# apelykh/deep-audio-mixer

Measured on AMD Instinct MI355X. Metric: stem-spectrogram-frames/sec (train), higher is better.
Workload: dtype f32; 1 GPU; C3: model_resnet (ResNet18, 8 stems) train step incl. STFT front-end, 8-stem 3 s @ 44.1 kHz stereo clips, n_fft 2048 hop 1024 -> 8x1025x130 per clip; batch_per_gpu=8, global_batch=8, parallelism=dp1, hip_graph=True, world_size=1, device_index=0, grad_buckets=1, allreduce_overlap=False

## Files before the change

### deep-audio-mixer_amd/csrc/dam_common.h

```cpp
#pragma once
#include <hip/hip_runtime.h>
#include <stdint.h>
#include "dam_hip.h"

#define DAM_CHECK_LAUNCH()                                   \
    do {                                                     \
        if (hipGetLastError() != hipSuccess) return DAM_ERR_LAUNCH; \
    } while (0)

namespace dam {

constexpr int WAVE = 64;

typedef float f32x4 __attribute__((ext_vector_type(4)));
typedef float f32x2 __attribute__((ext_vector_type(2)));
typedef float f32x4_u __attribute__((ext_vector_type(4), aligned(4)));
typedef double f64x2_u __attribute__((ext_vector_type(2), aligned(8)));

__device__ __forceinline__ float2 cmul(float2 a, float2 b) {
    return make_float2(a.x * b.x - a.y * b.y, a.x * b.y + a.y * b.x);
}
__device__ __forceinline__ float2 cadd(float2 a, float2 b) { return make_float2(a.x + b.x, a.y + b.y); }
__device__ __forceinline__ float2 csub(float2 a, float2 b) { return make_float2(a.x - b.x, a.y - b.y); }

__device__ __forceinline__ void wave_lds_sync() {
    __builtin_amdgcn_fence(__ATOMIC_RELEASE, "workgroup");
    __builtin_amdgcn_wave_barrier();
    __builtin_amdgcn_fence(__ATOMIC_ACQUIRE, "workgroup");
}

__device__ __forceinline__ void wave_lds_order() {
    asm volatile("s_waitcnt lgkmcnt(0)" ::: "memory");
    __builtin_amdgcn_wave_barrier();
}

__device__ __forceinline__ float wave_sum16(float v) {
    v += __shfl_xor(v, 1);
    v += __shfl_xor(v, 2);
    v += __shfl_xor(v, 4);
    v += __shfl_xor(v, 8);
    return v;
}
__device__ __forceinline__ float wave_sum64(float v) {
    v = wave_sum16(v);
    v += __shfl_xor(v, 16);
    v += __shfl_xor(v, 32);
    return v;
}

static inline int64_t cdiv(int64_t a, int64_t b) { return (a + b - 1) / b; }

constexpr int BN_RECORDS_MAX = 2048;
constexpr int BN_BWD_RECORDS_MAX = 1024;

struct BnFinArgs {
    const float* gamma;
    const float* beta;
    float* running_mean;
    float* running_var;
    long long* num_batches;
    float momentum, eps;
    float* save_mean;
    float* save_invstd;
    float* scale;
    float* shift;
};

__device__ __forceinline__ void store_sc1(float* p, float v) {
    __hip_atomic_store(p, v, __ATOMIC_RELAXED, __HIP_MEMORY_SCOPE_AGENT);
}

constexpr int MAX_DEVICES = 32;
static inline int device_slot() {
    int d = 0;
    if (hipGetDevice(&d) != hipSuccess || d < 0) d = 0;
    return d % MAX_DEVICES;
}
template <class T>
struct PerDevice {
    T v[MAX_DEVICES] = {};
    T& operator()() { return v[device_slot()]; }
};
template <auto Kernel>
static inline bool raise_lds_limit(int bytes) {
    static PerDevice<bool> raised_pd;
    bool& raised = raised_pd();
    if (!raised)
        raised = hipFuncSetAttribute(reinterpret_cast<const void*>(Kernel), hipFuncAttributeMaxDynamicSharedMemorySize, bytes) == hipSuccess;
    return raised;
}
static inline int device_cus() {
    static PerDevice<int> cus;
    int& n = cus();
    if (!n) {
        int dev = 0;
        if (hipGetDevice(&dev) != hipSuccess || hipDeviceGetAttribute(&n, hipDeviceAttributeMultiprocessorCount, dev) != hipSuccess || n < 1) n = 256;
    }
    return n;
}

}
```

### deep-audio-mixer_amd/csrc/dam_conv_s2.hip

```cpp
#include "dam_common.h"

namespace dam {
namespace {

typedef float v4f __attribute__((ext_vector_type(4)));

template <int NB, int NCH, bool STATS, int WAVES>
__global__ __launch_bounds__(64 * WAVES) void conv_s2_pair_kernel(const float* __restrict__ X, unsigned x_bytes, const float4* __restrict__ Wp,
                                                           const float4* __restrict__ Wp2, int Hd, int Wd, int H, int W,
                                                           float* __restrict__ Y, float* __restrict__ Ys, float* __restrict__ P1,
                                                           float* __restrict__ P2, int total_px, int total_units) {
    extern __shared__ __attribute__((aligned(16))) unsigned char smem[];
    constexpr int Ci = 16 * NCH, Co = 16 * NB;
    static_assert(NCH == 1 || NCH == 2, "the operand sets alternate per chunk (NCH == 2) or per unit (NCH == 1)");
    const int tid = threadIdx.x, lane = tid & 63, wave = tid >> 6;
    const int j = lane & 15, kq = lane >> 4;
    const __amdgpu_buffer_rsrc_t xr = __builtin_amdgcn_make_buffer_rsrc(const_cast<float*>(X), 0, x_bytes, 0x00020000);
    const int w_lane = lane * 16;
    float4 xs[2][9], wa[2][NB];
    v4f acc1[NB], accs[NB];
    float k1[STATS ? NB : 1][4], s11[STATS ? NB : 1][4], s21[STATS ? NB : 1][4];
    float ks[STATS ? NB : 1][4], s1s[STATS ? NB : 1][4], s2s[STATS ? NB : 1][4];
    int n_px = 0;
#pragma unroll
    for (int nb = 0; nb < NB; ++nb) {
        acc1[nb] = (v4f){0.f, 0.f, 0.f, 0.f};
        accs[nb] = (v4f){0.f, 0.f, 0.f, 0.f};
    }
    if constexpr (STATS) {
#pragma unroll
        for (int nb = 0; nb < NB; ++nb)
#pragma unroll
            for (int q = 0; q < 4; ++q) { k1[nb][q] = s11[nb][q] = s21[nb][q] = 0.f; ks[nb][q] = s1s[nb][q] = s2s[nb][q] = 0.f; }
    }
#define DAM_CS2_OFFS(U_, BASE_, FL_)                                                                                          \
    do {                                                                                                                      \
        const int p_ = (U_) * 16 + j;                                                                                         \
        const int row_ = p_ / Wd, col_ = p_ - row_ * Wd, img_ = row_ / Hd, i_ = row_ - img_ * Hd;                             \
        BASE_ = (((img_ * H + 2 * i_) * W + 2 * col_) * Ci + kq * 4) * 4;                                                     \
        FL_ = ((U_) < unit_end && p_ < total_px)                                                                             \
                  ? (1 | (i_ > 0 ? 2 : 0) | (2 * i_ + 1 < H ? 4 : 0) | (col_ > 0 ? 8 : 0) | (2 * col_ + 1 < W ? 16 : 0))      \
                  : 0;                                                                                                        \
    } while (0)
#define DAM_CS2_LOAD(S_, BASE_, FL_, CH_)                                                                                     \
    _Pragma("unroll") for (int a = 0; a < 3; ++a) {                                                                           \
        _Pragma("unroll") for (int b = 0; b < 3; ++b) {                                                                       \
            const int need = 1 | (a == 0 ? 2 : a == 2 ? 4 : 0) | (b == 0 ? 8 : b == 2 ? 16 : 0);                              \
            const int off = ((FL_) & need) == need ? (BASE_) + ((a - 1) * W + (b - 1)) * (Ci * 4) : 0x7fffffff;               \
            xs[S_][a * 3 + b] = __builtin_bit_cast(float4, __builtin_amdgcn_raw_buffer_load_b128(xr, off, (CH_) * 64, 0));    \
        }                                                                                                                     \
    }
#define DAM_CS2_MFMA4(ACC_, WA_, XV_)                                                                                         \
    do {                                                                                                                      \
        ACC_ = __builtin_amdgcn_mfma_f32_16x16x4f32(WA_.x, XV_.x, ACC_, 0, 0, 0);                                             \
        ACC_ = __builtin_amdgcn_mfma_f32_16x16x4f32(WA_.y, XV_.y, ACC_, 0, 0, 0);                                             \
        ACC_ = __builtin_amdgcn_mfma_f32_16x16x4f32(WA_.z, XV_.z, ACC_, 0, 0, 0);                                             \
        ACC_ = __builtin_amdgcn_mfma_f32_16x16x4f32(WA_.w, XV_.w, ACC_, 0, 0, 0);                                             \
    } while (0)
#define DAM_CS2_WREAD(BUF_, T_, CH_)                                                                                          \
    _Pragma("unroll") for (int nb = 0; nb < NB; ++nb)                                                                         \
        wa[BUF_][nb] = *reinterpret_cast<const float4*>(smem + w_lane + (((T_) * NCH + (CH_)) * NB + nb) * 1024);
#define DAM_CS2_COMPUTE(S_, CH_)                                                                                              \
    do {                                                                                                                      \
        DAM_CS2_WREAD(0, 0, CH_)                                                                                              \
        _Pragma("unroll") for (int t = 0; t < 10; ++t) {                                                                      \
            if (t < 9) { DAM_CS2_WREAD((t + 1) & 1, t + 1, CH_) }                                                             \
            __builtin_amdgcn_sched_barrier(0);                                                                                \
                                 \
            _Pragma("unroll") for (int q = 0; q < 4; ++q) {                                                                   \
                _Pragma("unroll") for (int nb = 0; nb < NB; ++nb) {                                                           \
                    const float wq = q == 0 ? wa[t & 1][nb].x : q == 1 ? wa[t & 1][nb].y : q == 2 ? wa[t & 1][nb].z : wa[t & 1][nb].w; \
                    const float4 xv = xs[S_][t < 9 ? t : 4];                                                                  \
                    const float xq = q == 0 ? xv.x : q == 1 ? xv.y : q == 2 ? xv.z : xv.w;                                    \
                    if (t < 9) acc1[nb] = __builtin_amdgcn_mfma_f32_16x16x4f32(wq, xq, acc1[nb], 0, 0, 0);                    \
                    else accs[nb] = __builtin_amdgcn_mfma_f32_16x16x4f32(wq, xq, accs[nb], 0, 0, 0);                          \
                }                                                                                                             \
            }                                                                                                                 \
            __builtin_amdgcn_sched_barrier(0);                                                                                \
        }                                                                                                                     \
    } while (0)
#define DAM_CS2_EPILOGUE(U_)                                                                                                  \
    do {                                                                                                                      \
        const int p_ = (U_) * 16 + j;                                                                                         \
        if (p_ < total_px) {                                                                                                  \
            float* o1 = Y + (size_t)p_ * Co + kq * 4;                                                                         \
            float* o2 = Ys + (size_t)p_ * Co + kq * 4;                                                                        \
            _Pragma("unroll") for (int nb = 0; nb < NB; ++nb) {                                                               \
                *reinterpret_cast<v4f*>(o1 + nb * 16) = acc1[nb];                                                             \
                *reinterpret_cast<v4f*>(o2 + nb * 16) = accs[nb];                                                             \
            }                                                                                                                 \
            if constexpr (STATS) {                                                                                            \
                _Pragma("unroll") for (int nb = 0; nb < NB; ++nb) {                                                           \
                    _Pragma("unroll") for (int q = 0; q < 4; ++q) {                                                           \
                        if (n_px == 0) { k1[nb][q] = acc1[nb][q]; ks[nb][q] = accs[nb][q]; }                                  \
                        const float d1 = acc1[nb][q] - k1[nb][q], d2 = accs[nb][q] - ks[nb][q];                               \
                        s11[nb][q] += d1; s21[nb][q] = fmaf(d1, d1, s21[nb][q]);                                              \
                        s1s[nb][q] += d2; s2s[nb][q] = fmaf(d2, d2, s2s[nb][q]);                                              \
                    }                                                                                                         \
                }                                                                                                             \
                ++n_px;                                                                                                       \
            }                                                                                                                 \
        }                                                                                                                     \
        _Pragma("unroll") for (int nb = 0; nb < NB; ++nb) {                                                                   \
            acc1[nb] = (v4f){0.f, 0.f, 0.f, 0.f};                                                                             \
            accs[nb] = (v4f){0.f, 0.f, 0.f, 0.f};                                                                             \
        }                                                                                                                     \
    } while (0)

    const int n_xcd = (gridDim.x & 7) == 0 ? 8 : 1;
    const int wg_per_xcd = gridDim.x / n_xcd, per_xcd = (total_units + n_xcd - 1) / n_xcd;
    const int u_lo = (blockIdx.x % n_xcd) * per_xcd;
    const int unit_end = u_lo + per_xcd < total_units ? u_lo + per_xcd : total_units;
    const int ustride = wg_per_xcd * WAVES;
    int unit = u_lo + wave * wg_per_xcd + blockIdx.x / n_xcd;
    int base0, fl0, base1, fl1;
    DAM_CS2_OFFS(unit, base0, fl0);
    DAM_CS2_LOAD(0, base0, fl0, 0)
    {
        constexpr int N4 = 9 * NCH * NB * 64, N4P = NCH * NB * 64;
        for (int e = tid; e < N4; e += 64 * WAVES) reinterpret_cast<float4*>(smem)[e] = Wp[e];
        for (int e = tid; e < N4P; e += 64 * WAVES) reinterpret_cast<float4*>(smem)[N4 + e] = Wp2[e];
    }
    __syncthreads();
    while (unit < unit_end) {
        if constexpr (NCH == 2) {
            DAM_CS2_LOAD(1, base0, fl0, 1)
            DAM_CS2_OFFS(unit + ustride, base1, fl1);
            __builtin_amdgcn_sched_barrier(0);
            DAM_CS2_COMPUTE(0, 0);
            __builtin_amdgcn_sched_barrier(0);
            DAM_CS2_LOAD(0, base1, fl1, 0)
            __builtin_amdgcn_sched_barrier(0);
            DAM_CS2_COMPUTE(1, 1);
            __builtin_amdgcn_sched_barrier(0);
            DAM_CS2_EPILOGUE(unit);
            unit += ustride;
            base0 = base1; fl0 = fl1;
        } else {
            const int u1 = unit + ustride, u2 = u1 + ustride;
            DAM_CS2_OFFS(u1, base1, fl1);
            DAM_CS2_LOAD(1, base1, fl1, 0)
            __builtin_amdgcn_sched_barrier(0);
            DAM_CS2_COMPUTE(0, 0);
            __builtin_amdgcn_sched_barrier(0);
            DAM_CS2_EPILOGUE(unit);
            DAM_CS2_OFFS(u2, base0, fl0);
            DAM_CS2_LOAD(0, base0, fl0, 0)
            __builtin_amdgcn_sched_barrier(0);
            if (u1 < unit_end) {
                DAM_CS2_COMPUTE(1, 0);
                __builtin_amdgcn_sched_barrier(0);
                DAM_CS2_EPILOGUE(u1);
            }
            unit = u2;
        }
    }
#undef DAM_CS2_OFFS
#undef DAM_CS2_LOAD
#undef DAM_CS2_MFMA4
#undef DAM_CS2_COMPUTE
#undef DAM_CS2_WREAD
#undef DAM_CS2_EPILOGUE
    if constexpr (STATS) {
        float cnt = (float)n_px;
        const float inv = n_px ? 1.0f / cnt : 0.f;
        float mean1[NB][4], m21[NB][4], means[NB][4], m2s[NB][4];
#pragma unroll
        for (int nb = 0; nb < NB; ++nb)
#pragma unroll
            for (int q = 0; q < 4; ++q) {
                const float a = s11[nb][q] * inv, b = s1s[nb][q] * inv;
                mean1[nb][q] = n_px ? k1[nb][q] + a : 0.f;
                m21[nb][q] = n_px ? fmaxf(s21[nb][q] - s11[nb][q] * a, 0.f) : 0.f;
                means[nb][q] = n_px ? ks[nb][q] + b : 0.f;
                m2s[nb][q] = n_px ? fmaxf(s2s[nb][q] - s1s[nb][q] * b, 0.f) : 0.f;
            }
#pragma unroll
        for (int off = 1; off < 16; off <<= 1) {
            const float cb = __shfl_xor(cnt, off), nn = cnt + cb;
            const float r = nn > 0.f ? cb / nn : 0.f, f = cnt * r;
#pragma unroll
            for (int nb = 0; nb < NB; ++nb)
#pragma unroll
                for (int q = 0; q < 4; ++q) {
                    float mb = __shfl_xor(mean1[nb][q], off), qb = __shfl_xor(m21[nb][q], off), d = mb - mean1[nb][q];
                    mean1[nb][q] = fmaf(d, r, mean1[nb][q]);
                    m21[nb][q] += qb + d * d * f;
                    mb = __shfl_xor(means[nb][q], off); qb = __shfl_xor(m2s[nb][q], off); d = mb - means[nb][q];
                    means[nb][q] = fmaf(d, r, means[nb][q]);
                    m2s[nb][q] += qb + d * d * f;
                }
            cnt = nn;
        }
        __syncthreads();
        float* rec = reinterpret_cast<float*>(smem);
        if (j == 0) {
#pragma unroll
            for (int nb = 0; nb < NB; ++nb)
#pragma unroll
                for (int q = 0; q < 4; ++q) {
                    float* o1 = rec + ((wave * 2 + 0) * Co + nb * 16 + kq * 4 + q) * 3;
                    float* o2 = rec + ((wave * 2 + 1) * Co + nb * 16 + kq * 4 + q) * 3;
                    o1[0] = cnt; o1[1] = mean1[nb][q]; o1[2] = m21[nb][q];
                    o2[0] = cnt; o2[1] = means[nb][q]; o2[2] = m2s[nb][q];
                }
        }
        __syncthreads();
        if (tid < 2 * Co) {
            const int which = tid / Co, c = tid - which * Co;
            float n = 0.f, mean = 0.f, m2 = 0.f;
#pragma unroll
            for (int w = 0; w < WAVES; ++w) {
                const float* r = rec + ((w * 2 + which) * Co + c) * 3;
                const float nb_ = r[0], nn = n + nb_, rr = nn > 0.f ? nb_ / nn : 0.f, d = r[1] - mean;
                mean = fmaf(d, rr, mean);
                m2 += r[2] + d * d * (n * rr);
                n = nn;
            }
            float* o = (which ? P2 : P1) + ((size_t)blockIdx.x * Co + c) * 3;
            o[0] = n; o[1] = mean; o[2] = m2;
        }
    }
}

template <int NB, int NCH, int WAVES>
int launch_conv_s2_pair(const float* x, const float* wp, const float* wp2, int B, int H, int W, float* y, float* ys, float* p1,
                        float* p2, int* parts_host, hipStream_t st) {
    const int Hd = (H + 1) / 2, Wd = (W + 1) / 2;
    const int64_t px = (int64_t)B * Hd * Wd, xb = (int64_t)B * H * W * NCH * 64;
    if (px >= (1ll << 26) || xb >= (1ll << 31)) return DAM_ERR_UNSUPPORTED;
    const int64_t units = cdiv(px, 16);
    const size_t lds = (size_t)10 * NCH * NB * 1024;
    const int cus = device_cus();
    const bool stats = p1 != nullptr;
    static PerDevice<int> occ[2];
    int& oc = occ[stats ? 1 : 0]();
    if (!oc) {
        int n = 0;
        const hipError_t e = stats ? hipOccupancyMaxActiveBlocksPerMultiprocessor(&n, conv_s2_pair_kernel<NB, NCH, true, WAVES>, 64 * WAVES, lds)
                                   : hipOccupancyMaxActiveBlocksPerMultiprocessor(&n, conv_s2_pair_kernel<NB, NCH, false, WAVES>, 64 * WAVES, lds);
        oc = (e == hipSuccess && n >= 1) ? n : 1;
    }
    int max_per_cu = oc;
    if (max_per_cu > 3) max_per_cu = 3;
    if (WAVES == 8) max_per_cu = 1;
    if (max_per_cu < 1) max_per_cu = 1;
    while (max_per_cu > 1 && (int64_t)cus * max_per_cu > BN_RECORDS_MAX) --max_per_cu;
    if ((int64_t)cus > BN_RECORDS_MAX) return DAM_ERR_UNSUPPORTED;
    int per_cu = 1;
    int64_t best = 0;
    for (int n = 1; n <= max_per_cu; ++n) {
        const int64_t cost = cdiv(units, (int64_t)WAVES * cus * n) * n * 100;
        if (n == 1 || cost * 100 <= best * 115) { best = n == 1 ? cost : (cost < best ? cost : best); per_cu = n; }
    }
    int64_t wgs = (int64_t)cus * per_cu;
    if (wgs > cdiv(units, WAVES)) wgs = cdiv(units, WAVES);
    if (parts_host) *parts_host = stats ? (int)wgs : 0;
    if (lds > 64 * 1024 && !(stats ? raise_lds_limit<&conv_s2_pair_kernel<NB, NCH, true, WAVES>>(160 * 1024)
                                   : raise_lds_limit<&conv_s2_pair_kernel<NB, NCH, false, WAVES>>(160 * 1024))) return DAM_ERR_LAUNCH;
    if (stats)
        hipLaunchKernelGGL((conv_s2_pair_kernel<NB, NCH, true, WAVES>), dim3((unsigned)wgs), dim3(64 * WAVES), lds, st, x, (unsigned)xb,
                           reinterpret_cast<const float4*>(wp), reinterpret_cast<const float4*>(wp2), Hd, Wd, H, W, y, ys, p1, p2, (int)px,
                           (int)units);
    else
        hipLaunchKernelGGL((conv_s2_pair_kernel<NB, NCH, false, WAVES>), dim3((unsigned)wgs), dim3(64 * WAVES), lds, st, x, (unsigned)xb,
                           reinterpret_cast<const float4*>(wp), reinterpret_cast<const float4*>(wp2), Hd, Wd, H, W, y, ys, p1, p2, (int)px,
                           (int)units);
    DAM_CHECK_LAUNCH();
    return DAM_OK;
}


template <bool STATS>
__global__ __launch_bounds__(256) void conv_s2_pair_stream_kernel(const float* __restrict__ X, unsigned x_bytes, const float4* __restrict__ Wp,
                                                                  const float4* __restrict__ Wp2, int Hd, int Wd, int H, int W, int NCH,
                                                                  int NB, float* __restrict__ Y, float* __restrict__ Ys,
                                                                  float* __restrict__ P1, float* __restrict__ P2, int total_px) {
    __shared__ float rec[4][2][16][3];
    const int tid = threadIdx.x, lane = tid & 63, wave = tid >> 6;
    const int j = lane & 15, kq = lane >> 4;
    constexpr int MB = 1;
    const int xcd = blockIdx.x & 7, seq = blockIdx.x >> 3;
    const int nb = seq % NB, pgroup = (seq / NB) * 8 + xcd;
    if (pgroup * (64 * MB) >= total_px) return;
    const int Ci = 16 * NCH, Co = 16 * NB;
    const __amdgpu_buffer_rsrc_t xr = __builtin_amdgcn_make_buffer_rsrc(const_cast<float*>(X), 0, x_bytes, 0x00020000);
    int pix[MB], off[MB][9];
#pragma unroll
    for (int mb = 0; mb < MB; ++mb) {
        const int p = ((pgroup * 4 + wave) * MB + mb) * 16 + j;
        pix[mb] = p;
        const int row = p / Wd, col = p - row * Wd, img = row / Hd, i = row - img * Hd;
        const int base = (((img * H + 2 * i) * W + 2 * col) * Ci + kq * 4) * 4;
        const int fl = p < total_px ? (1 | (i > 0 ? 2 : 0) | (2 * i + 1 < H ? 4 : 0) | (col > 0 ? 8 : 0) | (2 * col + 1 < W ? 16 : 0)) : 0;
#pragma unroll
        for (int a = 0; a < 3; ++a)
#pragma unroll
            for (int b = 0; b < 3; ++b) {
                const int need = 1 | (a == 0 ? 2 : a == 2 ? 4 : 0) | (b == 0 ? 8 : b == 2 ? 16 : 0);
                off[mb][a * 3 + b] = (fl & need) == need ? base + ((a - 1) * W + (b - 1)) * (Ci * 4) : 0x7fffffff;
            }
    }
    __shared__ float4 wbuf[2][10 * 64];
    float4 xs[2][MB][9], wa[2], wr0, wr1, wr2;
    const int we0 = tid, we1 = tid + 256, we2 = tid < 128 ? tid + 512 : 0;
#define DAM_CS2S_WSRC(E_, CH_)                                                                                               \
    ((E_) < 576 ? Wp + ((size_t)(((E_) >> 6) * NCH + (CH_)) * NB + nb) * 64 + ((E_) & 63)                                     \
                : Wp2 + ((size_t)(CH_) * NB + nb) * 64 + ((E_) & 63))
#define DAM_CS2S_WFETCH(CH_)                                                                                                  \
    do {                                                                                                                      \
        wr0 = *DAM_CS2S_WSRC(we0, CH_); wr1 = *DAM_CS2S_WSRC(we1, CH_); wr2 = *DAM_CS2S_WSRC(we2, CH_);                       \
    } while (0)
#define DAM_CS2S_WSTORE(BUF_)                                                                                                 \
    do {                                                                                                                      \
        wbuf[BUF_][we0] = wr0; wbuf[BUF_][we1] = wr1;                                                                         \
        if (tid < 128) wbuf[BUF_][we2] = wr2;                                                                                 \
    } while (0)
#define DAM_CS2S_XLOAD(S_, CH_)                                                                                               \
    _Pragma("unroll") for (int mb = 0; mb < MB; ++mb)                                                                         \
        _Pragma("unroll") for (int t = 0; t < 9; ++t)                                                                         \
            xs[S_][mb][t] = __builtin_bit_cast(float4, __builtin_amdgcn_raw_buffer_load_b128(xr, off[mb][t], (CH_) * 64, 0));
#define DAM_CS2S_CHUNK(S_, BUF_)                                                                                              \
    do {                                                                                                                      \
        wa[0] = wbuf[BUF_][lane];                                                                                             \
        _Pragma("unroll") for (int t = 0; t < 10; ++t) {                                                                      \
            if (t < 9) wa[(t + 1) & 1] = wbuf[BUF_][(t + 1) * 64 + lane];                                                     \
            __builtin_amdgcn_sched_barrier(0);                                                                                \
            const float4 w_ = wa[t & 1];                                                                                      \
            _Pragma("unroll") for (int mb = 0; mb < MB; ++mb) {                                                               \
                const float4 x_ = xs[S_][mb][t < 9 ? t : 4];                                                                  \
                if (t < 9) {                                                                                                  \
                    acc1[mb] = __builtin_amdgcn_mfma_f32_16x16x4f32(w_.x, x_.x, acc1[mb], 0, 0, 0);                           \
                    acc1[mb] = __builtin_amdgcn_mfma_f32_16x16x4f32(w_.y, x_.y, acc1[mb], 0, 0, 0);                           \
                    acc1[mb] = __builtin_amdgcn_mfma_f32_16x16x4f32(w_.z, x_.z, acc1[mb], 0, 0, 0);                           \
                    acc1[mb] = __builtin_amdgcn_mfma_f32_16x16x4f32(w_.w, x_.w, acc1[mb], 0, 0, 0);                           \
                } else {                                                                                                      \
                    accs[mb] = __builtin_amdgcn_mfma_f32_16x16x4f32(w_.x, x_.x, accs[mb], 0, 0, 0);                           \
                    accs[mb] = __builtin_amdgcn_mfma_f32_16x16x4f32(w_.y, x_.y, accs[mb], 0, 0, 0);                           \
                    accs[mb] = __builtin_amdgcn_mfma_f32_16x16x4f32(w_.z, x_.z, accs[mb], 0, 0, 0);                           \
                    accs[mb] = __builtin_amdgcn_mfma_f32_16x16x4f32(w_.w, x_.w, accs[mb], 0, 0, 0);                           \
                }                                                                                                             \
            }                                                                                                                 \
            __builtin_amdgcn_sched_barrier(0);                                                                                \
        }                                                                                                                     \
    } while (0)
    v4f acc1[MB], accs[MB];
#pragma unroll
    for (int mb = 0; mb < MB; ++mb) { acc1[mb] = (v4f){0.f, 0.f, 0.f, 0.f}; accs[mb] = (v4f){0.f, 0.f, 0.f, 0.f}; }
    DAM_CS2S_XLOAD(0, 0)
    DAM_CS2S_WFETCH(0);
    DAM_CS2S_WSTORE(0);
    __syncthreads();
    for (int c = 0; c < NCH; c += 2) {
        DAM_CS2S_XLOAD(1, c + 1)
        DAM_CS2S_WFETCH(c + 1);
        __builtin_amdgcn_sched_barrier(0);
        DAM_CS2S_CHUNK(0, 0);
        __builtin_amdgcn_sched_barrier(0);
        DAM_CS2S_WSTORE(1);
        __syncthreads();
        if (c + 2 < NCH) {
            DAM_CS2S_XLOAD(0, c + 2)
            DAM_CS2S_WFETCH(c + 2);
        }
        __builtin_amdgcn_sched_barrier(0);
        DAM_CS2S_CHUNK(1, 1);
        __builtin_amdgcn_sched_barrier(0);
        if (c + 2 < NCH) { DAM_CS2S_WSTORE(0); }
        __syncthreads();
    }
#undef DAM_CS2S_WSRC
#undef DAM_CS2S_WFETCH
#undef DAM_CS2S_WSTORE
#undef DAM_CS2S_XLOAD
#undef DAM_CS2S_CHUNK
#pragma unroll
    for (int mb = 0; mb < MB; ++mb)
        if (pix[mb] < total_px) {
            *reinterpret_cast<v4f*>(Y + (size_t)pix[mb] * Co + nb * 16 + kq * 4) = acc1[mb];
            *reinterpret_cast<v4f*>(Ys + (size_t)pix[mb] * Co + nb * 16 + kq * 4) = accs[mb];
        }
    if constexpr (STATS) {
        float cnt = 0.f;
#pragma unroll
        for (int mb = 0; mb < MB; ++mb) cnt += pix[mb] < total_px ? 1.f : 0.f;
#pragma unroll
        for (int o = 1; o < 16; o <<= 1) cnt += __shfl_xor(cnt, o);
        const float inv = cnt > 0.f ? 1.f / cnt : 0.f;
        float mean[2][4], m2[2][4];
#pragma unroll
        for (int q = 0; q < 4; ++q) {
            float s1 = 0.f, s2 = 0.f;
#pragma unroll
            for (int mb = 0; mb < MB; ++mb)
                if (pix[mb] < total_px) { s1 += acc1[mb][q]; s2 += accs[mb][q]; }
#pragma unroll
            for (int o = 1; o < 16; o <<= 1) { s1 += __shfl_xor(s1, o); s2 += __shfl_xor(s2, o); }
            mean[0][q] = s1 * inv; mean[1][q] = s2 * inv;
            float d1 = 0.f, d2 = 0.f;
#pragma unroll
            for (int mb = 0; mb < MB; ++mb)
                if (pix[mb] < total_px) {
                    const float e1 = acc1[mb][q] - mean[0][q], e2 = accs[mb][q] - mean[1][q];
                    d1 = fmaf(e1, e1, d1); d2 = fmaf(e2, e2, d2);
                }
#pragma unroll
            for (int o = 1; o < 16; o <<= 1) { d1 += __shfl_xor(d1, o); d2 += __shfl_xor(d2, o); }
            m2[0][q] = d1; m2[1][q] = d2;
        }
        if (j == 0) {
#pragma unroll
            for (int q = 0; q < 4; ++q) {
                rec[wave][0][kq * 4 + q][0] = cnt; rec[wave][0][kq * 4 + q][1] = mean[0][q]; rec[wave][0][kq * 4 + q][2] = m2[0][q];
                rec[wave][1][kq * 4 + q][0] = cnt; rec[wave][1][kq * 4 + q][1] = mean[1][q]; rec[wave][1][kq * 4 + q][2] = m2[1][q];
            }
        }
        __syncthreads();
        if (tid < 32) {
            const int which = tid >> 4, c = tid & 15;
            float n = 0.f, mu = 0.f, q2 = 0.f;
#pragma unroll
            for (int w = 0; w < 4; ++w) {
                const float nw = rec[w][which][c][0], nn = n + nw, rr = nn > 0.f ? nw / nn : 0.f, d = rec[w][which][c][1] - mu;
                mu = fmaf(d, rr, mu);
                q2 += rec[w][which][c][2] + d * d * (n * rr);
                n = nn;
            }
            float* o = (which ? P2 : P1) + ((size_t)pgroup * Co + nb * 16 + c) * 3;
            o[0] = n; o[1] = mu; o[2] = q2;
        }
    }
}

int launch_conv_s2_pair_stream(const float* x, const float* wp, const float* wp2, int B, int H, int W, int Ci, int Co, float* y, float* ys,
                               float* p1, float* p2, int* parts_host, hipStream_t st) {
    const int Hd = (H + 1) / 2, Wd = (W + 1) / 2, NCH = Ci / 16, NB = Co / 16;
    const int64_t px = (int64_t)B * Hd * Wd, xb = (int64_t)B * H * W * Ci * 4;
    const int64_t groups = cdiv(px, 64);
    if (px >= (1ll << 26) || xb >= (1ll << 31) || groups * NB >= (1ll << 31) || (int64_t)9 * Ci * Co * 4 >= (1ll << 31)) return DAM_ERR_UNSUPPORTED;
    const bool stats = p1 != nullptr;
    if (stats && groups > BN_RECORDS_MAX) return DAM_ERR_UNSUPPORTED;
    if (parts_host) *parts_host = stats ? (int)groups : 0;
    const dim3 grid((unsigned)(cdiv(groups, 8) * 8 * NB)), block(256);
#define DAM_CS2S_GO(ST_)                                                                                                        \
    hipLaunchKernelGGL((conv_s2_pair_stream_kernel<ST_>), grid, block, 0, st, x, (unsigned)xb, reinterpret_cast<const float4*>(wp), \
                       reinterpret_cast<const float4*>(wp2), Hd, Wd, H, W, NCH, NB, y, ys, p1, p2, (int)px)
    if (stats) DAM_CS2S_GO(true); else DAM_CS2S_GO(false);
#undef DAM_CS2S_GO
    DAM_CHECK_LAUNCH();
    return DAM_OK;
}

}
}

extern "C" int dam_conv_s2_pair_fwd_f32(const float* x, const float* w_packed, const float* wsc_packed, int B, int H, int W, int Ci,
                                        int Co, float* y, float* ysc, float* partial, float* partial_sc, int* parts_host,
                                        void* stream) {
    using namespace dam;
    if (!x || !w_packed || !wsc_packed || !y || !ysc || B <= 0 || H <= 0 || W <= 0) return DAM_ERR_BAD_ARG;
    if ((partial != nullptr) != (partial_sc != nullptr)) return DAM_ERR_BAD_ARG;
    if (partial && !parts_host) return DAM_ERR_BAD_ARG;
    hipStream_t st = (hipStream_t)stream;
    if (Ci == 16 && Co == 32) return launch_conv_s2_pair<2, 1, 4>(x, w_packed, wsc_packed, B, H, W, y, ysc, partial, partial_sc, parts_host, st);
    if (Ci == 32 && Co == 64) return launch_conv_s2_pair<4, 2, 8>(x, w_packed, wsc_packed, B, H, W, y, ysc, partial, partial_sc, parts_host, st);
    if (Ci % 32 == 0 && Co % 16 == 0)
        return launch_conv_s2_pair_stream(x, w_packed, wsc_packed, B, H, W, Ci, Co, y, ysc, partial, partial_sc, parts_host, st);
    return DAM_ERR_UNSUPPORTED;
}
```

### deep-audio-mixer_amd/csrc/dam_dgrad_s2.hip

```cpp
#include "dam_common.h"

namespace dam {
namespace {

typedef float v4f __attribute__((ext_vector_type(4)));

struct S2Sums {
    const float* u; const unsigned char* bits; const float* mean; const float* invstd; float* rec;
};
template <int NB, int NCH, int MB, bool PAIR, int WAVES, bool SUMS>
__global__ __launch_bounds__(64 * WAVES) void dgrad_s2_kernel(const float* __restrict__ DC, const float4* __restrict__ Wp,
                                                       const float* __restrict__ DS, const float4* __restrict__ Wp2, int B, int Hd,
                                                       int Wd, float* __restrict__ DX, int H, int W, int total_px, int total_units,
                                                       const S2Sums sums) {
    extern __shared__ __attribute__((aligned(16))) unsigned char smem[];
    constexpr int Co = 16 * NCH, Ci = 16 * NB;
    const int tid = threadIdx.x, lane = tid & 63, wave = tid >> 6;
    const int j = lane & 15, kq = lane >> 4;
    const __amdgpu_buffer_rsrc_t cr = __builtin_amdgcn_make_buffer_rsrc(const_cast<float*>(DC), 0, (unsigned)((size_t)B * Hd * Wd * Co * 4), 0x00020000);
    const __amdgpu_buffer_rsrc_t sr = __builtin_amdgcn_make_buffer_rsrc(const_cast<float*>(PAIR ? DS : DC), 0, (unsigned)((size_t)B * Hd * Wd * Co * 4), 0x00020000);
    const int w_lane = lane * 16;
    float su1[SUMS ? NB : 1][4], su2[SUMS ? NB : 1][4];
    float4 umu[SUMS ? NB : 1], uis[SUMS ? NB : 1];
    if constexpr (SUMS) {
#pragma unroll
        for (int nb = 0; nb < NB; ++nb) {
            umu[nb] = *reinterpret_cast<const float4*>(sums.mean + nb * 16 + kq * 4);
            uis[nb] = *reinterpret_cast<const float4*>(sums.invstd + nb * 16 + kq * 4);
#pragma unroll
            for (int q = 0; q < 4; ++q) su1[nb][q] = su2[nb][q] = 0.f;
        }
    }
    static_assert(NCH % 2 == 0, "chunk c of every unit uses operand set c & 1");
    float4 xo[2][PAIR ? 5 : 4][MB], wa[2][NB];
    int o00[MB], o01[MB], o10[MB], o11[MB], n00[MB], n01[MB], n10[MB], n11[MB];
#define DAM_S2_OFFSETS(U_, A_, B_, C_, D_)                                                                                    \
    do {                                                                                                                      \
        _Pragma("unroll") for (int mb = 0; mb < MB; ++mb) {                                                                   \
            const int p_ = (U_) * (16 * MB) + mb * 16 + j;              \
            const int row_ = p_ / Wd, col_ = p_ - row_ * Wd, i_ = row_ % Hd;                                                  \
            const int base = (p_ * Co + kq * 4) * 4;                                                                          \
            const bool c0 = (U_) < unit_end && p_ < total_px,    c1 = c0 && col_ + 1 < Wd, row1_ = i_ + 1 < Hd;               \
            A_[mb] = c0 ? base : 0x7fffffff;                                                                                  \
            B_[mb] = c1 ? base + Co * 4 : 0x7fffffff;                                                                         \
            C_[mb] = (c0 && row1_) ? base + Wd * Co * 4 : 0x7fffffff;                                                         \
            D_[mb] = (c1 && row1_) ? base + (Wd + 1) * Co * 4 : 0x7fffffff;                                                   \
        }                                                                                                                     \
    } while (0)
#define DAM_S2_LOAD(S_, A_, B_, C_, D_, CH_)                                                                                  \
    _Pragma("unroll") for (int mb = 0; mb < MB; ++mb) {                                                                       \
        xo[S_][0][mb] = __builtin_bit_cast(float4, __builtin_amdgcn_raw_buffer_load_b128(cr, A_[mb], (CH_) * 64, 0));         \
        xo[S_][1][mb] = __builtin_bit_cast(float4, __builtin_amdgcn_raw_buffer_load_b128(cr, B_[mb], (CH_) * 64, 0));         \
        xo[S_][2][mb] = __builtin_bit_cast(float4, __builtin_amdgcn_raw_buffer_load_b128(cr, C_[mb], (CH_) * 64, 0));         \
        xo[S_][3][mb] = __builtin_bit_cast(float4, __builtin_amdgcn_raw_buffer_load_b128(cr, D_[mb], (CH_) * 64, 0));         \
        if constexpr (PAIR) xo[S_][4][mb] = __builtin_bit_cast(float4, __builtin_amdgcn_raw_buffer_load_b128(sr, A_[mb], (CH_) * 64, 0)); \
    }
    constexpr int NT = PAIR ? 10 : 9;
    constexpr int TAPS[10][3] = {{4, 0, 0}, {3, 1, 1}, {5, 1, 0}, {1, 2, 2}, {7, 2, 0}, {0, 3, 3}, {2, 3, 2}, {6, 3, 1}, {8, 3, 0}, {9, 0, 4}};
#define DAM_S2_WREAD(BUF_, T_, CH_)                                                                                           \
    _Pragma("unroll") for (int nb = 0; nb < NB; ++nb)                                                                         \
        wa[BUF_][nb] = *reinterpret_cast<const float4*>(smem + w_lane + (((T_) * NCH + (CH_)) * NB + nb) * 1024);
#define DAM_S2_CHUNK(S_, CH_)                                                                                                 \
    do {                                                                                                                      \
        DAM_S2_WREAD(0, TAPS[0][0], CH_)                                                                                      \
        _Pragma("unroll") for (int s = 0; s < NT; ++s) {                                                                      \
            if (s + 1 < NT) { DAM_S2_WREAD((s + 1) & 1, TAPS[s + 1 < NT ? s + 1 : 0][0], CH_) }                               \
            __builtin_amdgcn_sched_barrier(0);                                                                                \
                           \
            _Pragma("unroll") for (int q = 0; q < 4; ++q) {                                                                   \
                _Pragma("unroll") for (int nb = 0; nb < NB; ++nb) {                                                           \
                    _Pragma("unroll") for (int mb = 0; mb < MB; ++mb) {                                                       \
                        v4f& a_ = acc[TAPS[s][1]][mb][nb];                                                                    \
                        const float4 w_ = wa[s & 1][nb], x_ = xo[S_][TAPS[s][2]][mb];                                         \
                        const float wq = q == 0 ? w_.x : q == 1 ? w_.y : q == 2 ? w_.z : w_.w;                                \
                        const float xq = q == 0 ? x_.x : q == 1 ? x_.y : q == 2 ? x_.z : x_.w;                                \
                        a_ = __builtin_amdgcn_mfma_f32_16x16x4f32(wq, xq, a_, 0, 0, 0);                                       \
                    }                                                                                                         \
                }                                                                                                             \
            }                                                                                                                 \
            __builtin_amdgcn_sched_barrier(0);                                                                                \
        }                                                                                                                     \
    } while (0)
    const int n_xcd = (gridDim.x & 7) == 0 ? 8 : 1;
    const int wg_per_xcd = gridDim.x / n_xcd, per_xcd = (total_units + n_xcd - 1) / n_xcd;
    const int u_lo = (blockIdx.x % n_xcd) * per_xcd;
    const int unit_end = u_lo + per_xcd < total_units ? u_lo + per_xcd : total_units;
    const int ustride = wg_per_xcd * WAVES;
    int unit = u_lo + wave * wg_per_xcd + blockIdx.x / n_xcd;
    DAM_S2_OFFSETS(unit, o00, o01, o10, o11);
    DAM_S2_LOAD(0, o00, o01, o10, o11, 0)
    {
        constexpr int N4 = 9 * NCH * NB * 64, N4P = PAIR ? NCH * NB * 64 : 0;
        for (int e = tid; e < N4; e += 64 * WAVES) reinterpret_cast<float4*>(smem)[e] = Wp[e];
        if constexpr (PAIR)
            for (int e = tid; e < N4P; e += 64 * WAVES) reinterpret_cast<float4*>(smem)[N4 + e] = Wp2[e];
    }
    __syncthreads();
    while (unit < unit_end) {
        v4f acc[4][MB][NB];
#pragma unroll
        for (int cl = 0; cl < 4; ++cl)
#pragma unroll
            for (int mb = 0; mb < MB; ++mb)
#pragma unroll
                for (int nb = 0; nb < NB; ++nb) acc[cl][mb][nb] = (v4f){0.f, 0.f, 0.f, 0.f};
        DAM_S2_OFFSETS(unit + ustride, n00, n01, n10, n11);
        float4 uv[SUMS ? MB : 1][4][NB];
        unsigned ub[SUMS ? MB : 1][4][NB];
#pragma unroll
        for (int c = 0; c < NCH; ++c) {
            if (c + 1 < NCH) { DAM_S2_LOAD((c + 1) & 1, o00, o01, o10, o11, c + 1) }
            else { DAM_S2_LOAD(0, n00, n01, n10, n11, 0) }
            if constexpr (SUMS) {
                if (c == NCH - 1) {
#pragma unroll
                    for (int mb = 0; mb < MB; ++mb) {
                        const int p = unit * (16 * MB) + mb * 16 + j;
                        const int row = p / Wd, col = p - row * Wd, img = row / Hd, i = row - img * Hd;
                        const bool live = p < total_px, orow1 = 2 * i + 1 < H, ocol1 = 2 * col + 1 < W;
                        const size_t px00 = ((size_t)img * H + 2 * i) * W + 2 * col;
#pragma unroll
                        for (int cl = 0; cl < 4; ++cl) {
                            const bool ok = live && (cl & 1 ? ocol1 : true) && (cl & 2 ? orow1 : true);
                            const size_t px = px00 + (cl & 1 ? 1 : 0) + (cl & 2 ? (size_t)W : 0);
#pragma unroll
                            for (int nb = 0; nb < NB; ++nb) {
                                uv[mb][cl][nb] = ok ? *reinterpret_cast<const float4*>(sums.u + px * Ci + nb * 16 + kq * 4) : make_float4(0.f, 0.f, 0.f, 0.f);
                                ub[mb][cl][nb] = ok ? sums.bits[px * (Ci / 4) + nb * 4 + kq] : 0u;
                            }
                        }
                    }
                }
            }
            __builtin_amdgcn_sched_barrier(0);
            DAM_S2_CHUNK(c & 1, c);
            __builtin_amdgcn_sched_barrier(0);
        }
#pragma unroll
        for (int mb = 0; mb < MB; ++mb) {
            const int p = unit * (16 * MB) + mb * 16 + j;
            if (p >= total_px) continue;
            const int row = p / Wd, col = p - row * Wd, img = row / Hd, i = row - img * Hd;
            const bool orow1 = 2 * i + 1 < H, ocol1 = 2 * col + 1 < W;
            const size_t px00 = ((size_t)img * H + 2 * i) * W + 2 * col;
            const size_t p00 = px00 * Ci + kq * 4;
            if constexpr (SUMS) {
#pragma unroll
                for (int nb = 0; nb < NB; ++nb) {
                    float* o = DX + p00 + nb * 16;
                    *reinterpret_cast<v4f*>(o) = acc[0][mb][nb];
                    if (ocol1) *reinterpret_cast<v4f*>(o + Ci) = acc[1][mb][nb];
                    if (orow1) {
                        *reinterpret_cast<v4f*>(o + (size_t)W * Ci) = acc[2][mb][nb];
                        if (ocol1) *reinterpret_cast<v4f*>(o + (size_t)W * Ci + Ci) = acc[3][mb][nb];
                    }
                }
#pragma unroll
                for (int cl = 0; cl < 4; ++cl)
#pragma unroll
                    for (int nb = 0; nb < NB; ++nb) {
                        const float uq[4] = {uv[mb][cl][nb].x, uv[mb][cl][nb].y, uv[mb][cl][nb].z, uv[mb][cl][nb].w};
                        const float mq[4] = {umu[nb].x, umu[nb].y, umu[nb].z, umu[nb].w}, iq[4] = {uis[nb].x, uis[nb].y, uis[nb].z, uis[nb].w};
#pragma unroll
                        for (int q = 0; q < 4; ++q) {
                            const float dz = (ub[mb][cl][nb] >> q) & 1u ? acc[cl][mb][nb][q] : 0.f;
                            su1[nb][q] += dz;
                            su2[nb][q] = fmaf(dz, (uq[q] - mq[q]) * iq[q], su2[nb][q]);
                        }
                    }
            } else {
#pragma unroll
                for (int nb = 0; nb < NB; ++nb) {
                    float* o = DX + p00 + nb * 16;
                    *reinterpret_cast<v4f*>(o) = acc[0][mb][nb];
                    if (ocol1) *reinterpret_cast<v4f*>(o + Ci) = acc[1][mb][nb];
                    if (orow1) {
                        *reinterpret_cast<v4f*>(o + (size_t)W * Ci) = acc[2][mb][nb];
                        if (ocol1) *reinterpret_cast<v4f*>(o + (size_t)W * Ci + Ci) = acc[3][mb][nb];
                    }
                }
            }
        }
        unit += ustride;
#pragma unroll
        for (int mb = 0; mb < MB; ++mb) { o00[mb] = n00[mb]; o01[mb] = n01[mb]; o10[mb] = n10[mb]; o11[mb] = n11[mb]; }
    }
    if constexpr (SUMS) {
#pragma unroll
        for (int off = 1; off < 16; off <<= 1)
#pragma unroll
            for (int nb = 0; nb < NB; ++nb)
#pragma unroll
                for (int q = 0; q < 4; ++q) { su1[nb][q] += __shfl_xor(su1[nb][q], off); su2[nb][q] += __shfl_xor(su2[nb][q], off); }
        __syncthreads();
        float* red = reinterpret_cast<float*>(smem);
        if (j == 0) {
#pragma unroll
            for (int nb = 0; nb < NB; ++nb)
#pragma unroll
                for (int q = 0; q < 4; ++q) {
                    red[(wave * Ci + nb * 16 + kq * 4 + q) * 2] = su1[nb][q];
                    red[(wave * Ci + nb * 16 + kq * 4 + q) * 2 + 1] = su2[nb][q];
                }
        }
        __syncthreads();
        if (tid < 2 * Ci) {
            float t = 0.f;
#pragma unroll
            for (int w = 0; w < WAVES; ++w) t += red[w * Ci * 2 + tid];
            sums.rec[(size_t)blockIdx.x * Ci * 2 + tid] = t;
        }
    }
#undef DAM_S2_OFFSETS
#undef DAM_S2_LOAD
#undef DAM_S2_WREAD
#undef DAM_S2_CHUNK
}

template <int NB, int NCH, int MB, int WAVES>
int launch_dgrad_s2(const float* dc, const float* wpt, const float* ds, const float* wpt2, int B, int Hd, int Wd, float* dx, int H,
                    int W, const S2Sums& sums, int* parts_host, hipStream_t st) {
    const int64_t px = (int64_t)B * Hd * Wd;
    if (px >= (1ll << 30)) return DAM_ERR_UNSUPPORTED;
    const int64_t units = cdiv(px, 16 * MB);
    const size_t lds = (size_t)(9 + (ds ? 1 : 0)) * NCH * NB * 1024;
    const int cus = device_cus();
    static PerDevice<int> occ[2][2];
    int& oc = occ[ds ? 1 : 0][sums.u ? 1 : 0]();
    if (!oc) {
        int n = 0;
        hipError_t e;
        if (ds) e = sums.u ? hipOccupancyMaxActiveBlocksPerMultiprocessor(&n, dgrad_s2_kernel<NB, NCH, MB, true, WAVES, true>, 64 * WAVES, lds)
                           : hipOccupancyMaxActiveBlocksPerMultiprocessor(&n, dgrad_s2_kernel<NB, NCH, MB, true, WAVES, false>, 64 * WAVES, lds);
        else e = sums.u ? hipOccupancyMaxActiveBlocksPerMultiprocessor(&n, dgrad_s2_kernel<NB, NCH, MB, false, WAVES, true>, 64 * WAVES, lds)
                        : hipOccupancyMaxActiveBlocksPerMultiprocessor(&n, dgrad_s2_kernel<NB, NCH, MB, false, WAVES, false>, 64 * WAVES, lds);
        oc = (e == hipSuccess && n >= 1) ? n : 1;
    }
    int max_per_cu = oc;
    if (max_per_cu > 3) max_per_cu = 3;
    if (WAVES == 8) max_per_cu = 1;
    int per_cu = 1;
    int64_t best = 0;
    for (int n = 1; n <= max_per_cu; ++n) {
        const int64_t cost = cdiv(units, (int64_t)WAVES * cus * n) * n * 100;
        if (n == 1 || cost * 100 <= best * 115) { best = n == 1 ? cost : (cost < best ? cost : best); per_cu = n; }
    }
    int64_t wgs = (int64_t)cus * per_cu;
    if (wgs > cdiv(units, WAVES)) wgs = cdiv(units, WAVES);
    if (sums.u && wgs > BN_BWD_RECORDS_MAX) return DAM_ERR_UNSUPPORTED;
#define DAM_S2_GO(PAIR_, SUMS_)                                                                                                   \
    do {                                                                                                                          \
        if (lds > 64 * 1024 && !raise_lds_limit<&dgrad_s2_kernel<NB, NCH, MB, PAIR_, WAVES, SUMS_>>(160 * 1024)) return DAM_ERR_LAUNCH; \
        hipLaunchKernelGGL((dgrad_s2_kernel<NB, NCH, MB, PAIR_, WAVES, SUMS_>), dim3((unsigned)wgs), dim3(64 * WAVES), lds, st, dc, \
                           reinterpret_cast<const float4*>(wpt), ds, reinterpret_cast<const float4*>(wpt2), B, Hd, Wd, dx, H, W,      \
                           (int)px, (int)units, sums);                                                                            \
    } while (0)
    if (ds) { if (sums.u) DAM_S2_GO(true, true); else DAM_S2_GO(true, false); }
    else { if (sums.u) DAM_S2_GO(false, true); else DAM_S2_GO(false, false); }
#undef DAM_S2_GO
    if (parts_host) *parts_host = sums.u ? (int)wgs : 0;
    DAM_CHECK_LAUNCH();
    return DAM_OK;
}


template <bool PAIR>
__global__ __launch_bounds__(256) void dgrad_s2_stream_kernel(const float* __restrict__ DC, const float4* __restrict__ Wp,
                                                              const float* __restrict__ DS, const float4* __restrict__ Wp2, int Hd, int Wd,
                                                              float* __restrict__ DX, int H, int W, int total_px, int NCH, int NB,
                                                              int total_units) {
    constexpr int MB = 2;
    const int lane = threadIdx.x & 63, wave = threadIdx.x >> 6;
    const int unit = blockIdx.x * 4 + wave;
    if (unit >= total_units) return;
    const int nb = unit % NB, pg = unit / NB;
    const int j = lane & 15, kq = lane >> 4;
    const int Co = 16 * NCH, Ci = 16 * NB;
    const __amdgpu_buffer_rsrc_t cr = __builtin_amdgcn_make_buffer_rsrc(const_cast<float*>(DC), 0, (unsigned)((size_t)total_px * Co * 4), 0x00020000);
    const __amdgpu_buffer_rsrc_t sr = __builtin_amdgcn_make_buffer_rsrc(const_cast<float*>(PAIR ? DS : DC), 0, (unsigned)((size_t)total_px * Co * 4), 0x00020000);
    const __amdgpu_buffer_rsrc_t wr = __builtin_amdgcn_make_buffer_rsrc(const_cast<float4*>(Wp), 0, (unsigned)((size_t)9 * NCH * NB * 1024), 0x00020000);
    const __amdgpu_buffer_rsrc_t w2r = __builtin_amdgcn_make_buffer_rsrc(const_cast<float4*>(PAIR ? Wp2 : Wp), 0, (unsigned)((size_t)NCH * NB * 1024), 0x00020000);
    int o00[MB], o01[MB], o10[MB], o11[MB];
#pragma unroll
    for (int mb = 0; mb < MB; ++mb) {
        const int p = pg * (16 * MB) + mb * 16 + j;
        const int row = p / Wd, col = p - row * Wd, i = row % Hd;
        const int base = (p * Co + kq * 4) * 4;
        const bool c0 = p < total_px, c1 = c0 && col + 1 < Wd, row1 = i + 1 < Hd;
        o00[mb] = c0 ? base : 0x7fffffff;
        o01[mb] = c1 ? base + Co * 4 : 0x7fffffff;
        o10[mb] = (c0 && row1) ? base + Wd * Co * 4 : 0x7fffffff;
        o11[mb] = (c1 && row1) ? base + (Wd + 1) * Co * 4 : 0x7fffffff;
    }
    float4 x00[2][MB], x01[2][MB], x10[2][MB], x11[2][MB], s00[2][PAIR ? MB : 1], wt[2][PAIR ? 10 : 9];
#define DAM_S2S_LOAD(S_, CH_)                                                                                                 \
    do {                                                                                                                      \
        _Pragma("unroll") for (int mb = 0; mb < MB; ++mb) {                                                                   \
            x00[S_][mb] = __builtin_bit_cast(float4, __builtin_amdgcn_raw_buffer_load_b128(cr, o00[mb], (CH_) * 64, 0));      \
            x01[S_][mb] = __builtin_bit_cast(float4, __builtin_amdgcn_raw_buffer_load_b128(cr, o01[mb], (CH_) * 64, 0));      \
            x10[S_][mb] = __builtin_bit_cast(float4, __builtin_amdgcn_raw_buffer_load_b128(cr, o10[mb], (CH_) * 64, 0));      \
            x11[S_][mb] = __builtin_bit_cast(float4, __builtin_amdgcn_raw_buffer_load_b128(cr, o11[mb], (CH_) * 64, 0));      \
            if constexpr (PAIR) s00[S_][mb] = __builtin_bit_cast(float4, __builtin_amdgcn_raw_buffer_load_b128(sr, o00[mb], (CH_) * 64, 0)); \
        }                                                                                                                     \
        _Pragma("unroll") for (int t = 0; t < 9; ++t)                                                                         \
            wt[S_][t] = __builtin_bit_cast(float4, __builtin_amdgcn_raw_buffer_load_b128(wr, lane * 16, ((t * NCH + (CH_)) * NB + nb) * 1024, 0)); \
        if constexpr (PAIR)                                                                                                   \
            wt[S_][9] = __builtin_bit_cast(float4, __builtin_amdgcn_raw_buffer_load_b128(w2r, lane * 16, ((CH_) * NB + nb) * 1024, 0)); \
    } while (0)
#define DAM_S2S_TAP(T_, CL_, X_, S_)                                                                                          \
    _Pragma("unroll") for (int mb = 0; mb < MB; ++mb) {                                                                       \
        acc[CL_][mb] = __builtin_amdgcn_mfma_f32_16x16x4f32(wt[S_][T_].x, X_[S_][mb].x, acc[CL_][mb], 0, 0, 0);               \
        acc[CL_][mb] = __builtin_amdgcn_mfma_f32_16x16x4f32(wt[S_][T_].y, X_[S_][mb].y, acc[CL_][mb], 0, 0, 0);               \
        acc[CL_][mb] = __builtin_amdgcn_mfma_f32_16x16x4f32(wt[S_][T_].z, X_[S_][mb].z, acc[CL_][mb], 0, 0, 0);               \
        acc[CL_][mb] = __builtin_amdgcn_mfma_f32_16x16x4f32(wt[S_][T_].w, X_[S_][mb].w, acc[CL_][mb], 0, 0, 0);               \
    }
#define DAM_S2S_CHUNK(S_)                                                                                                     \
    do {                                                                                                                      \
        DAM_S2S_TAP(4, 0, x00, S_)                                                                                            \
        if constexpr (PAIR) { DAM_S2S_TAP(9, 0, s00, S_) }                                                                    \
        DAM_S2S_TAP(3, 1, x01, S_) DAM_S2S_TAP(5, 1, x00, S_)                                                                 \
        DAM_S2S_TAP(1, 2, x10, S_) DAM_S2S_TAP(7, 2, x00, S_)                                                                 \
        DAM_S2S_TAP(0, 3, x11, S_) DAM_S2S_TAP(2, 3, x10, S_) DAM_S2S_TAP(6, 3, x01, S_) DAM_S2S_TAP(8, 3, x00, S_)           \
    } while (0)
    v4f acc[4][MB];
#pragma unroll
    for (int cl = 0; cl < 4; ++cl)
#pragma unroll
        for (int mb = 0; mb < MB; ++mb) acc[cl][mb] = (v4f){0.f, 0.f, 0.f, 0.f};
    DAM_S2S_LOAD(0, 0);
    for (int c = 0; c < NCH; c += 2) {
        DAM_S2S_LOAD(1, c + 1);
        __builtin_amdgcn_sched_barrier(0);
        DAM_S2S_CHUNK(0);
        __builtin_amdgcn_sched_barrier(0);
        if (c + 2 < NCH) DAM_S2S_LOAD(0, c + 2);
        __builtin_amdgcn_sched_barrier(0);
        DAM_S2S_CHUNK(1);
        __builtin_amdgcn_sched_barrier(0);
    }
#pragma unroll
    for (int mb = 0; mb < MB; ++mb) {
        const int p = pg * (16 * MB) + mb * 16 + j;
        if (p >= total_px) continue;
        const int row = p / Wd, col = p - row * Wd, img = row / Hd, i = row - img * Hd;
        const bool orow1 = 2 * i + 1 < H, ocol1 = 2 * col + 1 < W;
        float* o = DX + (((size_t)img * H + 2 * i) * W + 2 * col) * Ci + nb * 16 + kq * 4;
        *reinterpret_cast<v4f*>(o) = acc[0][mb];
        if (ocol1) *reinterpret_cast<v4f*>(o + Ci) = acc[1][mb];
        if (orow1) {
            *reinterpret_cast<v4f*>(o + (size_t)W * Ci) = acc[2][mb];
            if (ocol1) *reinterpret_cast<v4f*>(o + (size_t)W * Ci + Ci) = acc[3][mb];
        }
    }
#undef DAM_S2S_LOAD
#undef DAM_S2S_TAP
#undef DAM_S2S_CHUNK
}

template <bool PAIR>
__global__ __launch_bounds__(256) void dgrad_s2_stream_lds_kernel(const float* __restrict__ DC, const float4* __restrict__ Wp,
                                                                  const float* __restrict__ DS, const float4* __restrict__ Wp2, int Hd,
                                                                  int Wd, float* __restrict__ DX, int H, int W, int total_px, int NCH,
                                                                  int NB) {
    constexpr int NT = PAIR ? 10 : 9, NQ = NT * 64;
    __shared__ float4 wbuf[2][NQ];
    const int tid = threadIdx.x, lane = tid & 63, wave = tid >> 6;
    const int xcd = blockIdx.x & 7, seq = blockIdx.x >> 3;
    const int nb = seq % NB, grp = (seq / NB) * 8 + xcd;
    if (grp * 64 >= total_px) return;
    const int pg = grp * 4 + wave;
    const int j = lane & 15, kq = lane >> 4;
    const int Co = 16 * NCH, Ci = 16 * NB;
    const __amdgpu_buffer_rsrc_t cr = __builtin_amdgcn_make_buffer_rsrc(const_cast<float*>(DC), 0, (unsigned)((size_t)total_px * Co * 4), 0x00020000);
    const __amdgpu_buffer_rsrc_t sr = __builtin_amdgcn_make_buffer_rsrc(const_cast<float*>(PAIR ? DS : DC), 0, (unsigned)((size_t)total_px * Co * 4), 0x00020000);
    const int p = pg * 16 + j;
    const int row = p / Wd, col = p - row * Wd, img = row / Hd, i = row - img * Hd;
    int ov[4];
    {
        const int base = (p * Co + kq * 4) * 4;
        const bool c0 = p < total_px, c1 = c0 && col + 1 < Wd, row1 = i + 1 < Hd;
        ov[0] = c0 ? base : 0x7fffffff;
        ov[1] = c1 ? base + Co * 4 : 0x7fffffff;
        ov[2] = (c0 && row1) ? base + Wd * Co * 4 : 0x7fffffff;
        ov[3] = (c1 && row1) ? base + (Wd + 1) * Co * 4 : 0x7fffffff;
    }
    float4 xo[2][PAIR ? 5 : 4], wa[2], wr0, wr1, wr2;
    const int we0 = tid, we1 = tid + 256, we2 = tid + 512 < NQ ? tid + 512 : 0;
#define DAM_S2L_WSRC(E_, CH_)                                                                                                \
    ((E_) < 576 ? Wp + ((size_t)(((E_) >> 6) * NCH + (CH_)) * NB + nb) * 64 + ((E_) & 63)                                     \
                : Wp2 + ((size_t)(CH_) * NB + nb) * 64 + ((E_) & 63))
#define DAM_S2L_WFETCH(CH_)                                                                                                   \
    do {                                                                                                                      \
        wr0 = *DAM_S2L_WSRC(we0, CH_); wr1 = *DAM_S2L_WSRC(we1, CH_); wr2 = *DAM_S2L_WSRC(we2, CH_);                          \
    } while (0)
#define DAM_S2L_WSTORE(BUF_)                                                                                                  \
    do {                                                                                                                      \
        wbuf[BUF_][we0] = wr0; wbuf[BUF_][we1] = wr1;                                                                         \
        if (tid + 512 < NQ) wbuf[BUF_][we2] = wr2;                                                                            \
    } while (0)
#define DAM_S2L_XLOAD(S_, CH_)                                                                                                \
    do {                                                                                                                      \
        _Pragma("unroll") for (int v = 0; v < 4; ++v)                                                                         \
            xo[S_][v] = __builtin_bit_cast(float4, __builtin_amdgcn_raw_buffer_load_b128(cr, ov[v], (CH_) * 64, 0));          \
        if constexpr (PAIR) xo[S_][4] = __builtin_bit_cast(float4, __builtin_amdgcn_raw_buffer_load_b128(sr, ov[0], (CH_) * 64, 0)); \
    } while (0)
    constexpr int TAPS[10][3] = {{4, 0, 0}, {3, 1, 1}, {5, 1, 0}, {1, 2, 2}, {7, 2, 0}, {0, 3, 3}, {2, 3, 2}, {6, 3, 1}, {8, 3, 0}, {9, 0, 4}};
#define DAM_S2L_CHUNK(S_, BUF_)                                                                                               \
    do {                                                                                                                      \
        wa[0] = wbuf[BUF_][TAPS[0][0] * 64 + lane];                                                                           \
        _Pragma("unroll") for (int s = 0; s < NT; ++s) {                                                                      \
            if (s + 1 < NT) wa[(s + 1) & 1] = wbuf[BUF_][TAPS[s + 1 < NT ? s + 1 : 0][0] * 64 + lane];                        \
            __builtin_amdgcn_sched_barrier(0);                                                                                \
            const float4 w_ = wa[s & 1], x_ = xo[S_][TAPS[s][2]];                                                             \
            v4f& a_ = acc[TAPS[s][1]];                                                                                        \
            a_ = __builtin_amdgcn_mfma_f32_16x16x4f32(w_.x, x_.x, a_, 0, 0, 0);                                               \
            a_ = __builtin_amdgcn_mfma_f32_16x16x4f32(w_.y, x_.y, a_, 0, 0, 0);                                               \
            a_ = __builtin_amdgcn_mfma_f32_16x16x4f32(w_.z, x_.z, a_, 0, 0, 0);                                               \
            a_ = __builtin_amdgcn_mfma_f32_16x16x4f32(w_.w, x_.w, a_, 0, 0, 0);                                               \
            __builtin_amdgcn_sched_barrier(0);                                                                                \
        }                                                                                                                     \
    } while (0)
    v4f acc[4];
#pragma unroll
    for (int cl = 0; cl < 4; ++cl) acc[cl] = (v4f){0.f, 0.f, 0.f, 0.f};
    DAM_S2L_XLOAD(0, 0);
    DAM_S2L_WFETCH(0);
    DAM_S2L_WSTORE(0);
    __syncthreads();
    for (int c = 0; c < NCH; c += 2) {
        DAM_S2L_XLOAD(1, c + 1);
        DAM_S2L_WFETCH(c + 1);
        __builtin_amdgcn_sched_barrier(0);
        DAM_S2L_CHUNK(0, 0);
        __builtin_amdgcn_sched_barrier(0);
        DAM_S2L_WSTORE(1);
        __syncthreads();
        if (c + 2 < NCH) {
            DAM_S2L_XLOAD(0, c + 2);
            DAM_S2L_WFETCH(c + 2);
        }
        __builtin_amdgcn_sched_barrier(0);
        DAM_S2L_CHUNK(1, 1);
        __builtin_amdgcn_sched_barrier(0);
        if (c + 2 < NCH) { DAM_S2L_WSTORE(0); }
        __syncthreads();
    }
#undef DAM_S2L_WSRC
#undef DAM_S2L_WFETCH
#undef DAM_S2L_WSTORE
#undef DAM_S2L_XLOAD
#undef DAM_S2L_CHUNK
    if (p < total_px) {
        const bool orow1 = 2 * i + 1 < H, ocol1 = 2 * col + 1 < W;
        float* o = DX + (((size_t)img * H + 2 * i) * W + 2 * col) * Ci + nb * 16 + kq * 4;
        *reinterpret_cast<v4f*>(o) = acc[0];
        if (ocol1) *reinterpret_cast<v4f*>(o + Ci) = acc[1];
        if (orow1) {
            *reinterpret_cast<v4f*>(o + (size_t)W * Ci) = acc[2];
            if (ocol1) *reinterpret_cast<v4f*>(o + (size_t)W * Ci + Ci) = acc[3];
        }
    }
}

int launch_dgrad_s2_stream(const float* dc, const float* wpt, const float* ds, const float* wpt2, int B, int Hd, int Wd, int Co, int Ci,
                           float* dx, int H, int W, hipStream_t st) {
    const int64_t px = (int64_t)B * Hd * Wd;
    const int NCH = Co / 16, NB = Ci / 16;
    const int MB = cdiv(px, 16) * NB >= 8 * 1024 ? 2 : 1;
    const int64_t units = cdiv(px, 16 * MB) * NB;
    if (px >= (1ll << 26) || units >= (1ll << 30)) return DAM_ERR_UNSUPPORTED;
    if (MB == 1) {
        const dim3 grid_l((unsigned)(cdiv(cdiv(px, 64), 8) * 8 * NB)), block_l(256);
        if (ds)
            hipLaunchKernelGGL((dgrad_s2_stream_lds_kernel<true>), grid_l, block_l, 0, st, dc, reinterpret_cast<const float4*>(wpt), ds,
                               reinterpret_cast<const float4*>(wpt2), Hd, Wd, dx, H, W, (int)px, NCH, NB);
        else
            hipLaunchKernelGGL((dgrad_s2_stream_lds_kernel<false>), grid_l, block_l, 0, st, dc, reinterpret_cast<const float4*>(wpt),
                               (const float*)nullptr, (const float4*)nullptr, Hd, Wd, dx, H, W, (int)px, NCH, NB);
        DAM_CHECK_LAUNCH();
        return DAM_OK;
    }
    const dim3 grid((unsigned)cdiv(units, 4)), block(256);
    if (ds)
        hipLaunchKernelGGL((dgrad_s2_stream_kernel<true>), grid, block, 0, st, dc, reinterpret_cast<const float4*>(wpt), ds,
                           reinterpret_cast<const float4*>(wpt2), Hd, Wd, dx, H, W, (int)px, NCH, NB, (int)units);
    else
        hipLaunchKernelGGL((dgrad_s2_stream_kernel<false>), grid, block, 0, st, dc, reinterpret_cast<const float4*>(wpt),
                           (const float*)nullptr, (const float4*)nullptr, Hd, Wd, dx, H, W, (int)px, NCH, NB, (int)units);
    DAM_CHECK_LAUNCH();
    return DAM_OK;
}

}
}

extern "C" int dam_dgrad_s2_3x3_f32(const float* dy, const float* w_packed_t, const float* dy_pair, const float* w_pair_packed_t,
                                    int B, int Hd, int Wd, int Co, int Ci, float* dx, int H, int W, const dam_bn_bwd_sums* bn_bwd,
                                    float* bn_partial, int* bn_parts_host, void* stream) {
    using namespace dam;
    if (!dy || !w_packed_t || !dx || B <= 0 || Hd <= 0 || Wd <= 0 || H <= 0 || W <= 0) return DAM_ERR_BAD_ARG;
    if ((dy_pair != nullptr) != (w_pair_packed_t != nullptr)) return DAM_ERR_BAD_ARG;
    if (Hd != (H + 1) / 2 || Wd != (W + 1) / 2) return DAM_ERR_BAD_ARG;
    if ((int64_t)B * Hd * Wd * Co * 4 >= (1ll << 31)) return DAM_ERR_UNSUPPORTED;
    hipStream_t st = (hipStream_t)stream;
    if (bn_parts_host) *bn_parts_host = 0;
    S2Sums sums{nullptr, nullptr, nullptr, nullptr, nullptr};
    if (bn_bwd && bn_bwd->x && bn_bwd->mask_bits && bn_bwd->mean && bn_bwd->invstd && bn_partial && bn_parts_host)
        sums = S2Sums{bn_bwd->x, bn_bwd->mask_bits, bn_bwd->mean, bn_bwd->invstd, bn_partial};
    if (Co == 32 && Ci == 16) return launch_dgrad_s2<1, 2, 2, 4>(dy, w_packed_t, dy_pair, w_pair_packed_t, B, Hd, Wd, dx, H, W, sums, bn_parts_host, st);
    if (Co == 64 && Ci == 32) return launch_dgrad_s2<2, 4, 1, 8>(dy, w_packed_t, dy_pair, w_pair_packed_t, B, Hd, Wd, dx, H, W, sums, bn_parts_host, st);
    if (Co % 32 == 0 && Ci % 16 == 0 && (int64_t)9 * Co * Ci * 4 < (1ll << 31))
        return launch_dgrad_s2_stream(dy, w_packed_t, dy_pair, w_pair_packed_t, B, Hd, Wd, Co, Ci, dx, H, W, st);
    return DAM_ERR_UNSUPPORTED;
}
```

Before: 2.044 million stem-spectrogram-frames/s.

## Software-pipeline stride-2 conv kernels with deferred stores and magic-number division

Reworks the stride-2 conv forward and dgrad kernels. Output stores and BN-statistics updates for the previous unit are interleaved with the MFMA stream of the current unit using double-buffered accumulators and buffer stores. Accumulator zeroing is folded into the first MFMA, and integer divisions by Wd/Hd are replaced with precomputed multiply-high reciprocals. Pivot selection for statistics now uses DPP row broadcasts. This adds register pressure and scheduling complexity, and the dgrad launcher's size limits are tightened.

```diff
diff --git a/deep-audio-mixer_amd/csrc/dam_common.h b/deep-audio-mixer_amd/csrc/dam_common.h
--- a/deep-audio-mixer_amd/csrc/dam_common.h
+++ b/deep-audio-mixer_amd/csrc/dam_common.h
@@ -50,6 +50,17 @@
 
 static inline int64_t cdiv(int64_t a, int64_t b) { return (a + b - 1) / b; }
 
+struct MulHiDiv {
+    unsigned m, s;
+};
+static inline MulHiDiv mulhi_div(unsigned d) {
+    const unsigned D = 2u * d;
+    unsigned s = 0;
+    while ((2ull << s) < D) ++s;
+    return MulHiDiv{(unsigned)((1ull << (32 + s)) / D) + 1u, s};
+}
+__device__ __forceinline__ int mulhi_div(int n, MulHiDiv f) { return (int)(__umulhi(2u * (unsigned)n + 1u, f.m) >> f.s); }
+
 constexpr int BN_RECORDS_MAX = 2048;
 constexpr int BN_BWD_RECORDS_MAX = 1024;
 
diff --git a/deep-audio-mixer_amd/csrc/dam_conv_s2.hip b/deep-audio-mixer_amd/csrc/dam_conv_s2.hip
--- a/deep-audio-mixer_amd/csrc/dam_conv_s2.hip
+++ b/deep-audio-mixer_amd/csrc/dam_conv_s2.hip
@@ -4,29 +4,45 @@
 namespace {
 
 typedef float v4f __attribute__((ext_vector_type(4)));
+typedef int v4i __attribute__((ext_vector_type(4)));
+
+__device__ __forceinline__ float row_first(float v) {
+    return __builtin_bit_cast(float, __builtin_amdgcn_update_dpp(0, __builtin_bit_cast(int, v), 0x150, 0xF, 0xF, false));
+}
+__device__ __forceinline__ void row_sum(float& v) {
+    v += __builtin_bit_cast(float, __builtin_amdgcn_update_dpp(0, __builtin_bit_cast(int, v), 0x128, 0xF, 0xF, false));
+    v += __builtin_bit_cast(float, __builtin_amdgcn_update_dpp(0, __builtin_bit_cast(int, v), 0x124, 0xF, 0xF, false));
+    v += __builtin_bit_cast(float, __builtin_amdgcn_update_dpp(0, __builtin_bit_cast(int, v), 0x122, 0xF, 0xF, false));
+    v += __builtin_bit_cast(float, __builtin_amdgcn_update_dpp(0, __builtin_bit_cast(int, v), 0x121, 0xF, 0xF, false));
+}
 
 template <int NB, int NCH, bool STATS, int WAVES>
 __global__ __launch_bounds__(64 * WAVES) void conv_s2_pair_kernel(const float* __restrict__ X, unsigned x_bytes, const float4* __restrict__ Wp,
                                                            const float4* __restrict__ Wp2, int Hd, int Wd, int H, int W,
                                                            float* __restrict__ Y, float* __restrict__ Ys, float* __restrict__ P1,
-                                                           float* __restrict__ P2, int total_px, int total_units) {
+                                                           float* __restrict__ P2, int total_px, int total_units,
+                                                           const MulHiDiv div_wd, const MulHiDiv div_hd) {
     extern __shared__ __attribute__((aligned(16))) unsigned char smem[];
     constexpr int Ci = 16 * NCH, Co = 16 * NB;
     static_assert(NCH == 1 || NCH == 2, "the operand sets alternate per chunk (NCH == 2) or per unit (NCH == 1)");
-    const int tid = threadIdx.x, lane = tid & 63, wave = tid >> 6;
+    const int tid = threadIdx.x, lane = tid & 63, wave = __builtin_amdgcn_readfirstlane(tid >> 6);
     const int j = lane & 15, kq = lane >> 4;
     const __amdgpu_buffer_rsrc_t xr = __builtin_amdgcn_make_buffer_rsrc(const_cast<float*>(X), 0, x_bytes, 0x00020000);
     const int w_lane = lane * 16;
     float4 xs[2][9], wa[2][NB];
-    v4f acc1[NB], accs[NB];
+    constexpr int NSET = NCH == 1 ? 2 : 1;
+    v4f acc1[NSET][NB], accs[NSET][NB];
     float k1[STATS ? NB : 1][4], s11[STATS ? NB : 1][4], s21[STATS ? NB : 1][4];
     float ks[STATS ? NB : 1][4], s1s[STATS ? NB : 1][4], s2s[STATS ? NB : 1][4];
     int n_px = 0;
-#pragma unroll
-    for (int nb = 0; nb < NB; ++nb) {
-        acc1[nb] = (v4f){0.f, 0.f, 0.f, 0.f};
-        accs[nb] = (v4f){0.f, 0.f, 0.f, 0.f};
-    }
+    bool have_pivot = false;
+#pragma unroll
+    for (int nb = 0; nb < NB; ++nb)
+#pragma unroll
+        for (int a = 0; a < NSET; ++a) {
+            acc1[a][nb] = (v4f){0.f, 0.f, 0.f, 0.f};
+            accs[a][nb] = (v4f){0.f, 0.f, 0.f, 0.f};
+        }
     if constexpr (STATS) {
 #pragma unroll
         for (int nb = 0; nb < NB; ++nb)
@@ -36,7 +52,7 @@
 #define DAM_CS2_OFFS(U_, BASE_, FL_)                                                                                          \
     do {                                                                                                                      \
         const int p_ = (U_) * 16 + j;                                                                                         \
-        const int row_ = p_ / Wd, col_ = p_ - row_ * Wd, img_ = row_ / Hd, i_ = row_ - img_ * Hd;                             \
+        const int row_ = mulhi_div(p_, div_wd), col_ = p_ - row_ * Wd, img_ = mulhi_div(row_, div_hd), i_ = row_ - img_ * Hd; \
         BASE_ = (((img_ * H + 2 * i_) * W + 2 * col_) * Ci + kq * 4) * 4;                                                     \
         FL_ = ((U_) < unit_end && p_ < total_px)                                                                             \
                   ? (1 | (i_ > 0 ? 2 : 0) | (2 * i_ + 1 < H ? 4 : 0) | (col_ > 0 ? 8 : 0) | (2 * col_ + 1 < W ? 16 : 0))      \
@@ -72,8 +88,8 @@
                     const float wq = q == 0 ? wa[t & 1][nb].x : q == 1 ? wa[t & 1][nb].y : q == 2 ? wa[t & 1][nb].z : wa[t & 1][nb].w; \
                     const float4 xv = xs[S_][t < 9 ? t : 4];                                                                  \
                     const float xq = q == 0 ? xv.x : q == 1 ? xv.y : q == 2 ? xv.z : xv.w;                                    \
-                    if (t < 9) acc1[nb] = __builtin_amdgcn_mfma_f32_16x16x4f32(wq, xq, acc1[nb], 0, 0, 0);                    \
-                    else accs[nb] = __builtin_amdgcn_mfma_f32_16x16x4f32(wq, xq, accs[nb], 0, 0, 0);                          \
+                    if (t < 9) acc1[0][nb] = __builtin_amdgcn_mfma_f32_16x16x4f32(wq, xq, acc1[0][nb], 0, 0, 0);              \
+                    else accs[0][nb] = __builtin_amdgcn_mfma_f32_16x16x4f32(wq, xq, accs[0][nb], 0, 0, 0);                    \
                 }                                                                                                             \
             }                                                                                                                 \
             __builtin_amdgcn_sched_barrier(0);                                                                                \
@@ -82,18 +98,28 @@
 #define DAM_CS2_EPILOGUE(U_)                                                                                                  \
     do {                                                                                                                      \
         const int p_ = (U_) * 16 + j;                                                                                         \
+        if constexpr (STATS) {                                                                                                \
+            if (!have_pivot) {                      \
+                _Pragma("unroll") for (int nb = 0; nb < NB; ++nb) {                                                           \
+                    _Pragma("unroll") for (int q = 0; q < 4; ++q) {                                                           \
+                        k1[nb][q] = row_first(acc1[0][nb][q]);                                                                \
+                        ks[nb][q] = row_first(accs[0][nb][q]);                                                                \
+                    }                                                                                                         \
+                }                                                                                                             \
+                have_pivot = true;                                                                                            \
+            }                                                                                                                 \
+        }                                                                                                                     \
         if (p_ < total_px) {                                                                                                  \
             float* o1 = Y + (size_t)p_ * Co + kq * 4;                                                                         \
             float* o2 = Ys + (size_t)p_ * Co + kq * 4;                                                                        \
             _Pragma("unroll") for (int nb = 0; nb < NB; ++nb) {                                                               \
-                *reinterpret_cast<v4f*>(o1 + nb * 16) = acc1[nb];                                                             \
-                *reinterpret_cast<v4f*>(o2 + nb * 16) = accs[nb];                                                             \
+                *reinterpret_cast<v4f*>(o1 + nb * 16) = acc1[0][nb];                                                          \
+                *reinterpret_cast<v4f*>(o2 + nb * 16) = accs[0][nb];                                                          \
             }                                                                                                                 \
             if constexpr (STATS) {                                                                                            \
                 _Pragma("unroll") for (int nb = 0; nb < NB; ++nb) {                                                           \
                     _Pragma("unroll") for (int q = 0; q < 4; ++q) {                                                           \
-                        if (n_px == 0) { k1[nb][q] = acc1[nb][q]; ks[nb][q] = accs[nb][q]; }                                  \
-                        const float d1 = acc1[nb][q] - k1[nb][q], d2 = accs[nb][q] - ks[nb][q];                               \
+                        const float d1 = acc1[0][nb][q] - k1[nb][q], d2 = accs[0][nb][q] - ks[nb][q];                         \
                         s11[nb][q] += d1; s21[nb][q] = fmaf(d1, d1, s21[nb][q]);                                              \
                         s1s[nb][q] += d2; s2s[nb][q] = fmaf(d2, d2, s2s[nb][q]);                                              \
                     }                                                                                                         \
@@ -102,8 +128,8 @@
             }                                                                                                                 \
         }                                                                                                                     \
         _Pragma("unroll") for (int nb = 0; nb < NB; ++nb) {                                                                   \
-            acc1[nb] = (v4f){0.f, 0.f, 0.f, 0.f};                                                                             \
-            accs[nb] = (v4f){0.f, 0.f, 0.f, 0.f};                                                                             \
+            acc1[0][nb] = (v4f){0.f, 0.f, 0.f, 0.f};                                                                          \
+            accs[0][nb] = (v4f){0.f, 0.f, 0.f, 0.f};                                                                          \
         }                                                                                                                     \
     } while (0)
 
@@ -122,6 +148,104 @@
         for (int e = tid; e < N4P; e += 64 * WAVES) reinterpret_cast<float4*>(smem)[N4 + e] = Wp2[e];
     }
     __syncthreads();
+
+    const __amdgpu_buffer_rsrc_t yr = __builtin_amdgcn_make_buffer_rsrc(Y, 0, (unsigned)total_px * (Co * 4), 0x00020000);
+    const __amdgpu_buffer_rsrc_t ysr = __builtin_amdgcn_make_buffer_rsrc(Ys, 0, (unsigned)total_px * (Co * 4), 0x00020000);
+    int loff[9], bn = 0, fn = 0, e_off = 0x7fffffff;
+    bool e_live = false;
+#define DAM_CS2_TAPOFFS(BASE_, FL_)                                                                                           \
+    _Pragma("unroll") for (int a = 0; a < 3; ++a) {                                                                           \
+        _Pragma("unroll") for (int b = 0; b < 3; ++b) {                                                                       \
+            const int need = 1 | (a == 0 ? 2 : a == 2 ? 4 : 0) | (b == 0 ? 8 : b == 2 ? 16 : 0);                              \
+            loff[a * 3 + b] = ((FL_) & need) == need ? (BASE_) + ((a - 1) * W + (b - 1)) * (Ci * 4) : 0x7fffffff;             \
+        }                                                                                                                     \
+    }
+#define DAM_CS2_LOADX(S_)                                                                                                     \
+    _Pragma("unroll") for (int t = 0; t < 9; ++t)                                                                             \
+        xs[S_][t] = __builtin_bit_cast(float4, __builtin_amdgcn_raw_buffer_load_b128(xr, loff[t], 0, 0));
+#define DAM_CS2_STORES(PS_)                                                                                                   \
+    _Pragma("unroll") for (int nb = 0; nb < NB; ++nb) {                                                                       \
+        __builtin_amdgcn_raw_buffer_store_b128(__builtin_bit_cast(v4i, acc1[PS_][nb]), yr, e_off + nb * 64, 0, 0);                           \
+        __builtin_amdgcn_raw_buffer_store_b128(__builtin_bit_cast(v4i, accs[PS_][nb]), ysr, e_off + nb * 64, 0, 0);                          \
+    }
+#define DAM_CS2_STAT(PS_, V_)                                                                                                 \
+    do {                                                                                                                      \
+        const int nb_ = (V_) >> 2, q_ = (V_) & 3;                                                                             \
+        float d1 = acc1[PS_][nb_][q_] - k1[nb_][q_], d2 = accs[PS_][nb_][q_] - ks[nb_][q_];                                   \
+        d1 = e_live ? d1 : 0.f; d2 = e_live ? d2 : 0.f;                                                                       \
+        s11[nb_][q_] += d1; s21[nb_][q_] = fmaf(d1, d1, s21[nb_][q_]);                                                        \
+        s1s[nb_][q_] += d2; s2s[nb_][q_] = fmaf(d2, d2, s2s[nb_][q_]);                                                        \
+    } while (0)
+#define DAM_CS2_STREAM(S_, PS_, UNN_)                                                                                         \
+    do {                                                                                                                      \
+        DAM_CS2_WREAD(0, 0, 0)                                                                                                \
+        _Pragma("unroll") for (int t = 0; t < 10; ++t) {                                                                      \
+            if (t < 9) { DAM_CS2_WREAD((t + 1) & 1, t + 1, 0) }                                                               \
+            __builtin_amdgcn_sched_barrier(0);                                                                                \
+            _Pragma("unroll") for (int q = 0; q < 4; ++q) {                                                                   \
+                _Pragma("unroll") for (int nb = 0; nb < NB; ++nb) {                                                           \
+                    const float wq = q == 0 ? wa[t & 1][nb].x : q == 1 ? wa[t & 1][nb].y : q == 2 ? wa[t & 1][nb].z : wa[t & 1][nb].w; \
+                    const float4 xv = xs[S_][t < 9 ? t : 4];                                                                  \
+                    const float xq = q == 0 ? xv.x : q == 1 ? xv.y : q == 2 ? xv.z : xv.w;                                    \
+                    const v4f zero = {0.f, 0.f, 0.f, 0.f};                                                                    \
+                    if (t < 9) acc1[S_][nb] = __builtin_amdgcn_mfma_f32_16x16x4f32(wq, xq, t == 0 && q == 0 ? zero : acc1[S_][nb], 0, 0, 0); \
+                    else accs[S_][nb] = __builtin_amdgcn_mfma_f32_16x16x4f32(wq, xq, q == 0 ? zero : accs[S_][nb], 0, 0, 0);  \
+                }                                                                                                             \
+            }                                                                                                                 \
+            if (t == 0) {                                                                                                     \
+                DAM_CS2_STORES(PS_)                                                                                           \
+                if constexpr (STATS) n_px += e_live ? 1 : 0;                                                                  \
+            }                                                                                                                 \
+            if constexpr (STATS) {                                                                                            \
+                if (t < 8) {                                                                                                  \
+                    _Pragma("unroll") for (int v = t * (NB / 2); v < (t + 1) * (NB / 2); ++v) DAM_CS2_STAT(PS_, v);           \
+                }                                                                                                             \
+            }                                                                                                                 \
+                      \
+            if (t != 4) xs[S_][t == 9 ? 4 : t] = __builtin_bit_cast(float4, __builtin_amdgcn_raw_buffer_load_b128(xr, loff[t == 9 ? 4 : t], 0, 0)); \
+            if (t == 8) DAM_CS2_OFFS(UNN_, bn, fn);                                                                           \
+            if (t == 9) { DAM_CS2_TAPOFFS(bn, fn) }                                                                           \
+                            \
+            _Pragma("unroll") for (int m = 0; m < 4 * NB; ++m) {                                                              \
+                __builtin_amdgcn_sched_group_barrier(0x008, 1, 0);                                                            \
+                __builtin_amdgcn_sched_group_barrier(0x062, 4, 0);                                                            \
+            }                                                                                                                 \
+            __builtin_amdgcn_sched_barrier(0);                                                                                \
+        }                                                                                                                     \
+    } while (0)
+#define DAM_CS2_AFTER(S_, U_)                                                                                                 \
+    do {                                                                                                                      \
+        if constexpr (STATS) {                                                                                                \
+            if (!have_pivot) {                                                                                                \
+                _Pragma("unroll") for (int nb = 0; nb < NB; ++nb) {                                                           \
+                    _Pragma("unroll") for (int q = 0; q < 4; ++q) {                                                           \
+                        k1[nb][q] = row_first(acc1[S_][nb][q]);                                                               \
+                        ks[nb][q] = row_first(accs[S_][nb][q]);                                                               \
+                    }                                                                                                         \
+                }                                                                                                             \
+                have_pivot = true;                                                                                            \
+            }                                                                                                                 \
+        }                                                                                                                     \
+        const int p_ = (U_) * 16 + j;                                                                                         \
+        e_live = p_ < total_px;                                                                                               \
+        e_off = e_live ? (p_ * Co + kq * 4) * 4 : 0x7fffffff;                                                                 \
+    } while (0)
+#define DAM_CS2_DRAIN(PS_)                                                                                                    \
+    do {                                                                                                                      \
+        DAM_CS2_STORES(PS_)                                                                                                   \
+        if constexpr (STATS) {                                                                                                \
+            n_px += e_live ? 1 : 0;                                                                                           \
+            _Pragma("unroll") for (int v = 0; v < 4 * NB; ++v) DAM_CS2_STAT(PS_, v);                                          \
+        }                                                                                                                     \
+    } while (0)
+    if constexpr (NCH == 1) {
+        static_assert(NB % 2 == 0, "DAM_CS2_STREAM spreads the 4 * NB statistics channels over taps 0-7");
+        DAM_CS2_OFFS(unit + ustride, bn, fn);
+        DAM_CS2_TAPOFFS(bn, fn)
+        DAM_CS2_LOADX(1)
+        DAM_CS2_OFFS(unit + 2 * ustride, bn, fn);
+        DAM_CS2_TAPOFFS(bn, fn)
+    }
     while (unit < unit_end) {
         if constexpr (NCH == 2) {
             DAM_CS2_LOAD(1, base0, fl0, 1)
@@ -137,22 +261,14 @@
             unit += ustride;
             base0 = base1; fl0 = fl1;
         } else {
-            const int u1 = unit + ustride, u2 = u1 + ustride;
-            DAM_CS2_OFFS(u1, base1, fl1);
-            DAM_CS2_LOAD(1, base1, fl1, 0)
-            __builtin_amdgcn_sched_barrier(0);
-            DAM_CS2_COMPUTE(0, 0);
-            __builtin_amdgcn_sched_barrier(0);
-            DAM_CS2_EPILOGUE(unit);
-            DAM_CS2_OFFS(u2, base0, fl0);
-            DAM_CS2_LOAD(0, base0, fl0, 0)
-            __builtin_amdgcn_sched_barrier(0);
-            if (u1 < unit_end) {
-                DAM_CS2_COMPUTE(1, 0);
-                __builtin_amdgcn_sched_barrier(0);
-                DAM_CS2_EPILOGUE(u1);
-            }
-            unit = u2;
+            DAM_CS2_STREAM(0, 1, unit + 3 * ustride);
+            DAM_CS2_AFTER(0, unit);
+            unit += ustride;
+            if (unit >= unit_end) { DAM_CS2_DRAIN(0); break; }
+            DAM_CS2_STREAM(1, 0, unit + 3 * ustride);
+            DAM_CS2_AFTER(1, unit);
+            unit += ustride;
+            if (unit >= unit_end) { DAM_CS2_DRAIN(1); break; }
         }
     }
 #undef DAM_CS2_OFFS
@@ -161,37 +277,30 @@
 #undef DAM_CS2_COMPUTE
 #undef DAM_CS2_WREAD
 #undef DAM_CS2_EPILOGUE
+#undef DAM_CS2_TAPOFFS
+#undef DAM_CS2_LOADX
+#undef DAM_CS2_STORES
+#undef DAM_CS2_STAT
+#undef DAM_CS2_STREAM
+#undef DAM_CS2_AFTER
+#undef DAM_CS2_DRAIN
     if constexpr (STATS) {
         float cnt = (float)n_px;
-        const float inv = n_px ? 1.0f / cnt : 0.f;
+        row_sum(cnt);
+        const float inv = cnt > 0.f ? 1.0f / cnt : 0.f;
         float mean1[NB][4], m21[NB][4], means[NB][4], m2s[NB][4];
 #pragma unroll
         for (int nb = 0; nb < NB; ++nb)
 #pragma unroll
             for (int q = 0; q < 4; ++q) {
+                row_sum(s11[nb][q]); row_sum(s21[nb][q]);
+                row_sum(s1s[nb][q]); row_sum(s2s[nb][q]);
                 const float a = s11[nb][q] * inv, b = s1s[nb][q] * inv;
-                mean1[nb][q] = n_px ? k1[nb][q] + a : 0.f;
-                m21[nb][q] = n_px ? fmaxf(s21[nb][q] - s11[nb][q] * a, 0.f) : 0.f;
-                means[nb][q] = n_px ? ks[nb][q] + b : 0.f;
-                m2s[nb][q] = n_px ? fmaxf(s2s[nb][q] - s1s[nb][q] * b, 0.f) : 0.f;
+                mean1[nb][q] = k1[nb][q] + a;
+                m21[nb][q] = fmaxf(s21[nb][q] - s11[nb][q] * a, 0.f);
+                means[nb][q] = ks[nb][q] + b;
+                m2s[nb][q] = fmaxf(s2s[nb][q] - s1s[nb][q] * b, 0.f);
             }
-#pragma unroll
-        for (int off = 1; off < 16; off <<= 1) {
-            const float cb = __shfl_xor(cnt, off), nn = cnt + cb;
-            const float r = nn > 0.f ? cb / nn : 0.f, f = cnt * r;
-#pragma unroll
-            for (int nb = 0; nb < NB; ++nb)
-#pragma unroll
-                for (int q = 0; q < 4; ++q) {
-                    float mb = __shfl_xor(mean1[nb][q], off), qb = __shfl_xor(m21[nb][q], off), d = mb - mean1[nb][q];
-                    mean1[nb][q] = fmaf(d, r, mean1[nb][q]);
-                    m21[nb][q] += qb + d * d * f;
-                    mb = __shfl_xor(means[nb][q], off); qb = __shfl_xor(m2s[nb][q], off); d = mb - means[nb][q];
-                    means[nb][q] = fmaf(d, r, means[nb][q]);
-                    m2s[nb][q] += qb + d * d * f;
-                }
-            cnt = nn;
-        }
         __syncthreads();
         float* rec = reinterpret_cast<float*>(smem);
         if (j == 0) {
@@ -228,7 +337,7 @@
                         float* p2, int* parts_host, hipStream_t st) {
     const int Hd = (H + 1) / 2, Wd = (W + 1) / 2;
     const int64_t px = (int64_t)B * Hd * Wd, xb = (int64_t)B * H * W * NCH * 64;
-    if (px >= (1ll << 26) || xb >= (1ll << 31)) return DAM_ERR_UNSUPPORTED;
+    if (px >= (1ll << 26) || xb >= (1ll << 31) || px * NB * 64 >= (1ll << 31)) return DAM_ERR_UNSUPPORTED;
     const int64_t units = cdiv(px, 16);
     const size_t lds = (size_t)10 * NCH * NB * 1024;
     const int cus = device_cus();
@@ -261,11 +370,11 @@
     if (stats)
         hipLaunchKernelGGL((conv_s2_pair_kernel<NB, NCH, true, WAVES>), dim3((unsigned)wgs), dim3(64 * WAVES), lds, st, x, (unsigned)xb,
                            reinterpret_cast<const float4*>(wp), reinterpret_cast<const float4*>(wp2), Hd, Wd, H, W, y, ys, p1, p2, (int)px,
-                           (int)units);
+                           (int)units, mulhi_div((unsigned)Wd), mulhi_div((unsigned)Hd));
     else
         hipLaunchKernelGGL((conv_s2_pair_kernel<NB, NCH, false, WAVES>), dim3((unsigned)wgs), dim3(64 * WAVES), lds, st, x, (unsigned)xb,
                            reinterpret_cast<const float4*>(wp), reinterpret_cast<const float4*>(wp2), Hd, Wd, H, W, y, ys, p1, p2, (int)px,
-                           (int)units);
+                           (int)units, mulhi_div((unsigned)Wd), mulhi_div((unsigned)Hd));
     DAM_CHECK_LAUNCH();
     return DAM_OK;
 }
diff --git a/deep-audio-mixer_amd/csrc/dam_dgrad_s2.hip b/deep-audio-mixer_amd/csrc/dam_dgrad_s2.hip
--- a/deep-audio-mixer_amd/csrc/dam_dgrad_s2.hip
+++ b/deep-audio-mixer_amd/csrc/dam_dgrad_s2.hip
@@ -4,6 +4,7 @@
 namespace {
 
 typedef float v4f __attribute__((ext_vector_type(4)));
+typedef int v4i __attribute__((ext_vector_type(4)));
 
 struct S2Sums {
     const float* u; const unsigned char* bits; const float* mean; const float* invstd; float* rec;
@@ -12,10 +13,10 @@
 __global__ __launch_bounds__(64 * WAVES) void dgrad_s2_kernel(const float* __restrict__ DC, const float4* __restrict__ Wp,
                                                        const float* __restrict__ DS, const float4* __restrict__ Wp2, int B, int Hd,
                                                        int Wd, float* __restrict__ DX, int H, int W, int total_px, int total_units,
-                                                       const S2Sums sums) {
+                                                       const MulHiDiv div_wd, const MulHiDiv div_hd, const S2Sums sums) {
     extern __shared__ __attribute__((aligned(16))) unsigned char smem[];
     constexpr int Co = 16 * NCH, Ci = 16 * NB;
-    const int tid = threadIdx.x, lane = tid & 63, wave = tid >> 6;
+    const int tid = threadIdx.x, lane = tid & 63, wave = __builtin_amdgcn_readfirstlane(tid >> 6);
     const int j = lane & 15, kq = lane >> 4;
     const __amdgpu_buffer_rsrc_t cr = __builtin_amdgcn_make_buffer_rsrc(const_cast<float*>(DC), 0, (unsigned)((size_t)B * Hd * Wd * Co * 4), 0x00020000);
     const __amdgpu_buffer_rsrc_t sr = __builtin_amdgcn_make_buffer_rsrc(const_cast<float*>(PAIR ? DS : DC), 0, (unsigned)((size_t)B * Hd * Wd * Co * 4), 0x00020000);
@@ -34,12 +35,15 @@
     static_assert(NCH % 2 == 0, "chunk c of every unit uses operand set c & 1");
     float4 xo[2][PAIR ? 5 : 4][MB], wa[2][NB];
     int o00[MB], o01[MB], o10[MB], o11[MB], n00[MB], n01[MB], n10[MB], n11[MB];
-#define DAM_S2_OFFSETS(U_, A_, B_, C_, D_)                                                                                    \
+    int opx[MB], ofl[MB], npx[MB], nfl[MB];
+#define DAM_S2_OFFSETS(U_, A_, B_, C_, D_, PX_, FL_)                                                                          \
     do {                                                                                                                      \
         _Pragma("unroll") for (int mb = 0; mb < MB; ++mb) {                                                                   \
             const int p_ = (U_) * (16 * MB) + mb * 16 + j;              \
-            const int row_ = p_ / Wd, col_ = p_ - row_ * Wd, i_ = row_ % Hd;                                                  \
+            const int row_ = mulhi_div(p_, div_wd), col_ = p_ - row_ * Wd, img_ = mulhi_div(row_, div_hd), i_ = row_ - img_ * Hd; \
             const int base = (p_ * Co + kq * 4) * 4;                                                                          \
+            PX_[mb] = (img_ * H + 2 * i_) * W + 2 * col_;                                                                     \
+            FL_[mb] = (p_ < total_px ? 1 : 0) | (2 * col_ + 1 < W ? 2 : 0) | (2 * i_ + 1 < H ? 4 : 0);                        \
             const bool c0 = (U_) < unit_end && p_ < total_px,    c1 = c0 && col_ + 1 < Wd, row1_ = i_ + 1 < Hd;               \
             A_[mb] = c0 ? base : 0x7fffffff;                                                                                  \
             B_[mb] = c1 ? base + Co * 4 : 0x7fffffff;                                                                         \
@@ -56,27 +60,57 @@
         if constexpr (PAIR) xo[S_][4][mb] = __builtin_bit_cast(float4, __builtin_amdgcn_raw_buffer_load_b128(sr, A_[mb], (CH_) * 64, 0)); \
     }
     constexpr int NT = PAIR ? 10 : 9;
-    constexpr int TAPS[10][3] = {{4, 0, 0}, {3, 1, 1}, {5, 1, 0}, {1, 2, 2}, {7, 2, 0}, {0, 3, 3}, {2, 3, 2}, {6, 3, 1}, {8, 3, 0}, {9, 0, 4}};
+    constexpr int TAPS[10][3] = {{4, 0, 0}, {9, 0, 4}, {3, 1, 1}, {5, 1, 0}, {1, 2, 2}, {7, 2, 0}, {0, 3, 3}, {2, 3, 2}, {6, 3, 1}, {8, 3, 0}};
+    constexpr int T0 = PAIR ? 0 : 1;
+#define DAM_S2_TAP(S_, K_) (TAPS[(S_) == 0 ? 0 : (S_) + T0][K_])
+    static_assert(MB * NB == 2, "DAM_S2_FILL gives each of a class's MB * NB accumulators one of the two taps behind the class");
+    const __amdgpu_buffer_rsrc_t dxr = __builtin_amdgcn_make_buffer_rsrc(DX, 0, (unsigned)((size_t)B * H * W * Ci * 4), 0x00020000);
+#define DAM_S2_ITEM(CL_, MB_, NB_)                                                                                            \
+    do {                                                                                                                      \
+        const int need_ = 1 | ((CL_) & 1 ? 2 : 0) | ((CL_) & 2 ? 4 : 0);                                                      \
+        const int wo_ = (ofl[MB_] & need_) == need_                                                                           \
+                            ? (opx[MB_] + ((CL_) & 1 ? 1 : 0) + ((CL_) & 2 ? W : 0)) * (Ci * 4) + kq * 16 + (NB_) * 64        \
+                            : 0x7fffffff;                                                                                     \
+        __builtin_amdgcn_raw_buffer_store_b128(__builtin_bit_cast(v4i, acc[CL_][MB_][NB_]), dxr, wo_, 0, 0);                  \
+    } while (0)
+#define DAM_S2_FILL(s, CH_)                                                                                                   \
+    if ((CH_) == 0 && s == 0) DAM_S2_OFFSETS(unit + ustride, n00, n01, n10, n11, npx, nfl);                                   \
+    if ((CH_) == NCH - 1) {                                                                                                   \
+        _Pragma("unroll") for (int cl = 0; cl < 3; ++cl) {                                                                    \
+            const int it = s - ((PAIR ? 1 : 0) + 2 * cl) - 1;                                                                 \
+            if (it == 0) DAM_S2_ITEM(cl, 0, 0);                                                                               \
+            if (it == 1) DAM_S2_ITEM(cl, MB - 1, NB - 1);                                                                     \
+        }                                                                                                                     \
+    }
 #define DAM_S2_WREAD(BUF_, T_, CH_)                                                                                           \
     _Pragma("unroll") for (int nb = 0; nb < NB; ++nb)                                                                         \
         wa[BUF_][nb] = *reinterpret_cast<const float4*>(smem + w_lane + (((T_) * NCH + (CH_)) * NB + nb) * 1024);
 #define DAM_S2_CHUNK(S_, CH_)                                                                                                 \
     do {                                                                                                                      \
-        DAM_S2_WREAD(0, TAPS[0][0], CH_)                                                                                      \
+        DAM_S2_WREAD(0, DAM_S2_TAP(0, 0), CH_)                                                                                \
         _Pragma("unroll") for (int s = 0; s < NT; ++s) {                                                                      \
-            if (s + 1 < NT) { DAM_S2_WREAD((s + 1) & 1, TAPS[s + 1 < NT ? s + 1 : 0][0], CH_) }                               \
+            if (s + 1 < NT) { DAM_S2_WREAD((s + 1) & 1, DAM_S2_TAP(s + 1 < NT ? s + 1 : 0, 0), CH_) }                         \
             __builtin_amdgcn_sched_barrier(0);                                                                                \
-                           \
+             \
+                                                                 \
             _Pragma("unroll") for (int q = 0; q < 4; ++q) {                                                                   \
                 _Pragma("unroll") for (int nb = 0; nb < NB; ++nb) {                                                           \
                     _Pragma("unroll") for (int mb = 0; mb < MB; ++mb) {                                                       \
-                        v4f& a_ = acc[TAPS[s][1]][mb][nb];                                                                    \
-                        const float4 w_ = wa[s & 1][nb], x_ = xo[S_][TAPS[s][2]][mb];                                         \
+                        v4f& a_ = acc[DAM_S2_TAP(s, 1)][mb][nb];                                                              \
+                        const float4 w_ = wa[s & 1][nb], x_ = xo[S_][DAM_S2_TAP(s, 2)][mb];                                   \
                         const float wq = q == 0 ? w_.x : q == 1 ? w_.y : q == 2 ? w_.z : w_.w;                                \
                         const float xq = q == 0 ? x_.x : q == 1 ? x_.y : q == 2 ? x_.z : x_.w;                                \
-                        a_ = __builtin_amdgcn_mfma_f32_16x16x4f32(wq, xq, a_, 0, 0, 0);                                       \
+                        const bool first_ = (CH_) == 0 && q == 0 && (s == 0 || DAM_S2_TAP(s, 1) != DAM_S2_TAP(s > 0 ? s - 1 : 0, 1)); \
+                        const v4f zero_ = {0.f, 0.f, 0.f, 0.f};                                                               \
+                        a_ = __builtin_amdgcn_mfma_f32_16x16x4f32(wq, xq, first_ ? zero_ : a_, 0, 0, 0);                      \
                     }                                                                                                         \
                 }                                                                                                             \
+            }                                                                                                                 \
+            DAM_S2_FILL(s, CH_)                                                                                               \
+                            \
+            _Pragma("unroll") for (int m = 0; m < 4 * MB * NB; ++m) {                                                         \
+                __builtin_amdgcn_sched_group_barrier(0x008, 1, 0);                                                            \
+                __builtin_amdgcn_sched_group_barrier(0x042, 5, 0);                                                            \
             }                                                                                                                 \
             __builtin_amdgcn_sched_barrier(0);                                                                                \
         }                                                                                                                     \
@@ -87,7 +121,7 @@
     const int unit_end = u_lo + per_xcd < total_units ? u_lo + per_xcd : total_units;
     const int ustride = wg_per_xcd * WAVES;
     int unit = u_lo + wave * wg_per_xcd + blockIdx.x / n_xcd;
-    DAM_S2_OFFSETS(unit, o00, o01, o10, o11);
+    DAM_S2_OFFSETS(unit, o00, o01, o10, o11, opx, ofl);
     DAM_S2_LOAD(0, o00, o01, o10, o11, 0)
     {
         constexpr int N4 = 9 * NCH * NB * 64, N4P = PAIR ? NCH * NB * 64 : 0;
@@ -98,13 +132,6 @@
     __syncthreads();
     while (unit < unit_end) {
         v4f acc[4][MB][NB];
-#pragma unroll
-        for (int cl = 0; cl < 4; ++cl)
-#pragma unroll
-            for (int mb = 0; mb < MB; ++mb)
-#pragma unroll
-                for (int nb = 0; nb < NB; ++nb) acc[cl][mb][nb] = (v4f){0.f, 0.f, 0.f, 0.f};
-        DAM_S2_OFFSETS(unit + ustride, n00, n01, n10, n11);
         float4 uv[SUMS ? MB : 1][4][NB];
         unsigned ub[SUMS ? MB : 1][4][NB];
 #pragma unroll
@@ -115,10 +142,8 @@
                 if (c == NCH - 1) {
 #pragma unroll
                     for (int mb = 0; mb < MB; ++mb) {
-                        const int p = unit * (16 * MB) + mb * 16 + j;
-                        const int row = p / Wd, col = p - row * Wd, img = row / Hd, i = row - img * Hd;
-                        const bool live = p < total_px, orow1 = 2 * i + 1 < H, ocol1 = 2 * col + 1 < W;
-                        const size_t px00 = ((size_t)img * H + 2 * i) * W + 2 * col;
+                        const bool live = ofl[mb] & 1, ocol1 = ofl[mb] & 2, orow1 = ofl[mb] & 4;
+                        const size_t px00 = (size_t)opx[mb];
 #pragma unroll
                         for (int cl = 0; cl < 4; ++cl) {
                             const bool ok = live && (cl & 1 ? ocol1 : true) && (cl & 2 ? orow1 : true);
@@ -137,24 +162,12 @@
             __builtin_amdgcn_sched_barrier(0);
         }
 #pragma unroll
-        for (int mb = 0; mb < MB; ++mb) {
-            const int p = unit * (16 * MB) + mb * 16 + j;
-            if (p >= total_px) continue;
-            const int row = p / Wd, col = p - row * Wd, img = row / Hd, i = row - img * Hd;
-            const bool orow1 = 2 * i + 1 < H, ocol1 = 2 * col + 1 < W;
-            const size_t px00 = ((size_t)img * H + 2 * i) * W + 2 * col;
-            const size_t p00 = px00 * Ci + kq * 4;
-            if constexpr (SUMS) {
-#pragma unroll
-                for (int nb = 0; nb < NB; ++nb) {
-                    float* o = DX + p00 + nb * 16;
-                    *reinterpret_cast<v4f*>(o) = acc[0][mb][nb];
-                    if (ocol1) *reinterpret_cast<v4f*>(o + Ci) = acc[1][mb][nb];
-                    if (orow1) {
-                        *reinterpret_cast<v4f*>(o + (size_t)W * Ci) = acc[2][mb][nb];
-                        if (ocol1) *reinterpret_cast<v4f*>(o + (size_t)W * Ci + Ci) = acc[3][mb][nb];
-                    }
-                }
+        for (int mb = 0; mb < MB; ++mb)
+#pragma unroll
+            for (int nb = 0; nb < NB; ++nb) DAM_S2_ITEM(3, mb, nb);
+        if constexpr (SUMS) {
+#pragma unroll
+            for (int mb = 0; mb < MB; ++mb)
 #pragma unroll
                 for (int cl = 0; cl < 4; ++cl)
 #pragma unroll
@@ -168,22 +181,13 @@
                             su2[nb][q] = fmaf(dz, (uq[q] - mq[q]) * iq[q], su2[nb][q]);
                         }
                     }
-            } else {
-#pragma unroll
-                for (int nb = 0; nb < NB; ++nb) {
-                    float* o = DX + p00 + nb * 16;
-                    *reinterpret_cast<v4f*>(o) = acc[0][mb][nb];
-                    if (ocol1) *reinterpret_cast<v4f*>(o + Ci) = acc[1][mb][nb];
-                    if (orow1) {
-                        *reinterpret_cast<v4f*>(o + (size_t)W * Ci) = acc[2][mb][nb];
-                        if (ocol1) *reinterpret_cast<v4f*>(o + (size_t)W * Ci + Ci) = acc[3][mb][nb];
-                    }
-                }
-            }
         }
         unit += ustride;
 #pragma unroll
-        for (int mb = 0; mb < MB; ++mb) { o00[mb] = n00[mb]; o01[mb] = n01[mb]; o10[mb] = n10[mb]; o11[mb] = n11[mb]; }
+        for (int mb = 0; mb < MB; ++mb) {
+            o00[mb] = n00[mb]; o01[mb] = n01[mb]; o10[mb] = n10[mb]; o11[mb] = n11[mb];
+            opx[mb] = npx[mb]; ofl[mb] = nfl[mb];
+        }
     }
     if constexpr (SUMS) {
 #pragma unroll
@@ -215,13 +219,16 @@
 #undef DAM_S2_LOAD
 #undef DAM_S2_WREAD
 #undef DAM_S2_CHUNK
+#undef DAM_S2_TAP
+#undef DAM_S2_ITEM
+#undef DAM_S2_FILL
 }
 
 template <int NB, int NCH, int MB, int WAVES>
 int launch_dgrad_s2(const float* dc, const float* wpt, const float* ds, const float* wpt2, int B, int Hd, int Wd, float* dx, int H,
                     int W, const S2Sums& sums, int* parts_host, hipStream_t st) {
     const int64_t px = (int64_t)B * Hd * Wd;
-    if (px >= (1ll << 30)) return DAM_ERR_UNSUPPORTED;
+    if (px >= (1ll << 26) || (int64_t)B * H * W * NB * 64 >= (1ll << 31)) return DAM_ERR_UNSUPPORTED;
     const int64_t units = cdiv(px, 16 * MB);
     const size_t lds = (size_t)(9 + (ds ? 1 : 0)) * NCH * NB * 1024;
     const int cus = device_cus();
@@ -253,7 +260,7 @@
         if (lds > 64 * 1024 && !raise_lds_limit<&dgrad_s2_kernel<NB, NCH, MB, PAIR_, WAVES, SUMS_>>(160 * 1024)) return DAM_ERR_LAUNCH; \
         hipLaunchKernelGGL((dgrad_s2_kernel<NB, NCH, MB, PAIR_, WAVES, SUMS_>), dim3((unsigned)wgs), dim3(64 * WAVES), lds, st, dc, \
                            reinterpret_cast<const float4*>(wpt), ds, reinterpret_cast<const float4*>(wpt2), B, Hd, Wd, dx, H, W,      \
-                           (int)px, (int)units, sums);                                                                            \
+                           (int)px, (int)units, mulhi_div((unsigned)Wd), mulhi_div((unsigned)Hd), sums);                                                                            \
     } while (0)
     if (ds) { if (sums.u) DAM_S2_GO(true, true); else DAM_S2_GO(true, false); }
     else { if (sums.u) DAM_S2_GO(false, true); else DAM_S2_GO(false, false); }
```

Result: no change. 2.049 million stem-spectrogram-frames/s, median of 6 (+0.3%).
